# TrevorS/voxtral-mini-realtime-rs

Measured on AMD Instinct MI355X. Metric: decode_tok_per_s, higher is better.
Workload: dtype f32

## Files before the change

### include/voxtral_hip.h

```cpp
#ifndef VOXTRAL_HIP_H
#define VOXTRAL_HIP_H

#include <stddef.h>
#include <stdint.h>

#ifdef __cplusplus
extern "C" {
#endif

#define VOX_OK 0
#define VOX_ERR_INVALID 1
#define VOX_ERR_IO 2
#define VOX_ERR_HIP 3
#define VOX_ERR_NOTFOUND 4
#define VOX_ERR_UNSUPPORTED 5

#define VOX_MEM_HOST 0
#define VOX_MEM_DEVICE 1

typedef struct vox_ctx vox_ctx;
typedef struct vox_gguf vox_gguf;
typedef struct vox_q4 vox_q4;
typedef struct vox_model vox_model;
typedef struct vox_cache vox_cache;
// ... 14 lines not shown
int32_t vox_dev_download(vox_ctx* ctx, void* dst_host, const void* src_dev, size_t nbytes);
int32_t vox_dev_copy(vox_ctx* ctx, void* dst_dev, const void* src_dev, size_t nbytes);

int32_t vox_resample_len(size_t n_in, uint32_t sr_in, uint32_t sr_out, size_t* n_out);
int32_t vox_resample(vox_ctx* ctx, const float* in, size_t n_in, uint32_t sr_in, uint32_t sr_out, float* out, size_t cap, size_t* n_out,
                     int32_t mem_kind);
int32_t vox_resample_plan(uint32_t sr_in, uint32_t sr_out, int32_t* fft_in, int32_t* fft_out, int32_t* delay, float* cutoff, float* taps_or_null, size_t cap);
int32_t vox_peak_normalize(float* samples, size_t n, float target_peak);

typedef struct {
    uint32_t sample_rate;
    uint32_t n_left_pad_tokens;
    float    frame_rate;
    uint32_t extra_right_pad_tokens;
} vox_pad_cfg;
int32_t vox_pad_cfg_voxtral(vox_pad_cfg* cfg);
int32_t vox_pad_len(size_t n, const vox_pad_cfg* cfg, size_t* out);
int32_t vox_pad_audio(const float* in, size_t n, const vox_pad_cfg* cfg, float* out);
int32_t vox_num_audio_tokens(size_t n, const vox_pad_cfg* cfg, size_t* out);

typedef struct {
    uint32_t max_mel_frames;
    uint32_t hop_length;
    uint32_t sample_rate;
    uint32_t overlap_frames;
} vox_chunk_cfg;
typedef struct { size_t start_sample, end_sample, index; int32_t is_last; } vox_chunk;
int32_t vox_needs_chunking(size_t n, const vox_chunk_cfg* cfg, int32_t* out);
int32_t vox_chunk_plan(size_t n, const vox_chunk_cfg* cfg, vox_chunk* out, size_t cap, size_t* n_chunks);

int32_t vox_mel_num_frames(size_t n_samples, size_t* out);
int32_t vox_mel_filterbank(float* out_128x201);
int32_t vox_hann_window(int32_t length, float* out);
int32_t vox_mel_compute_log(vox_ctx* ctx, const float* samples, size_t n, float* out_Tx128, int32_t mem_kind);

int32_t vox_time_embedding(float t, int32_t dim, float* out);

int32_t vox_gguf_open(const char* path, vox_gguf** out);
int32_t vox_gguf_open_memory(const void* data, size_t size, vox_gguf** out);
int32_t vox_gguf_open_shards(const void* const* shards, const size_t* sizes, int32_t n, vox_gguf** out);
int32_t vox_gguf_close(vox_gguf* g);
int32_t vox_gguf_version(const vox_gguf* g, uint32_t* out);
int32_t vox_gguf_tensor_count(const vox_gguf* g, uint64_t* out);
int32_t vox_gguf_tensor_name(const vox_gguf* g, uint64_t index, const char** out);
int32_t vox_gguf_tensor_info(const vox_gguf* g, const char* name, uint64_t dims[4], uint32_t* ndims,
                             uint32_t* dtype, uint64_t* nbytes);
int32_t vox_gguf_tensor_data(const vox_gguf* g, const char* name, void* dst, size_t cap);

int32_t vox_q4_tensor_from_bytes(vox_ctx* ctx, const uint8_t* raw, size_t nbytes, int64_t N, int64_t K, vox_q4** out);
int32_t vox_q4_tensor_shape(const vox_q4* q, int64_t* N, int64_t* K);
int32_t vox_q4_tensor_num_blocks(const vox_q4* q, int64_t* out);
int32_t vox_q4_tensor_dequantize(vox_ctx* ctx, const vox_q4* q, float* out_NxK);
int32_t vox_q4_tensor_free(vox_q4* q);
int32_t vox_q4_matmul(vox_ctx* ctx, const vox_q4* w, const float* x, int32_t B, int32_t M, float* out, int32_t mem_kind);
int32_t vox_q4_linear_forward(vox_ctx* ctx, const vox_q4* w, const float* bias_or_null, const float* x,
                              int32_t B, int32_t M, float* out, int32_t mem_kind);

int32_t vox_dense_tensor_from_f32(vox_ctx* ctx, const float* w_NxK, const float* w_other_or_null, int64_t N, int64_t K, vox_q4** out);
int32_t vox_linear_forward_ex(vox_ctx* ctx, const vox_q4* w, const float* bias_or_null, const float* x, int32_t B, int32_t M, float* out, int32_t epilogue, int32_t mem_kind);
int32_t vox_conv_downsample(vox_ctx* ctx, const float* x_CxL, int32_t C, int32_t L, const float* w1, const float* b1, const float* w2, const float* b2, int32_t O, float* out_OxL2);

typedef struct {
    int32_t enc_layers, enc_dim, enc_heads, enc_head_dim, enc_ffn, enc_window;
    int32_t dec_layers, dec_dim, dec_heads, dec_kv_heads, dec_head_dim, dec_ffn, dec_window, vocab;
    int32_t n_mels, reshape_factor, t_cond_dim;
    float rope_theta, norm_eps;
} vox_model_cfg;

int32_t vox_attention(vox_ctx* ctx, const float* q, const float* k, const float* v, int32_t M, int32_t kv_len, int32_t n_heads,
                      int32_t n_kv_heads, int32_t head_dim, int32_t offset, int32_t window, float* out, int32_t mem_kind);

int32_t vox_q4_model_load(vox_ctx* ctx, const char* gguf_path, vox_model** out);
#define VOX_LOAD_LAYOUT_ONLY 1u
int32_t vox_q4_model_load_ex(vox_ctx* ctx, const char* gguf_path, uint32_t flags, vox_model** out);
int32_t vox_q4_model_load_gguf(vox_ctx* ctx, vox_gguf* g, uint32_t flags, vox_model** out);
int32_t vox_f32_model_load(vox_ctx* ctx, const char* safetensors_path, vox_model** out);
int32_t vox_model_free(vox_model* m);
int32_t vox_model_config(const vox_model* m, vox_model_cfg* out);
int32_t vox_model_weight_bytes(const vox_model* m, uint64_t* out);
int32_t vox_model_arena(const vox_model* m, void** dev_ptr, uint64_t* nbytes);
int32_t vox_model_arena_finalize(vox_model* m);
int32_t vox_model_replicate(const vox_model* src, vox_ctx* dst_ctx, vox_model** out);
int32_t vox_model_memory(const vox_model* m, uint64_t out[4]);

int32_t vox_model_set_t_embed(vox_model* m, const float* t_embed_host);
int32_t vox_model_set_decode_engine(vox_model* m, int32_t on, int32_t* active_or_null);
int32_t vox_model_set_prefix_cache(vox_model* m, int32_t on, int32_t* active_or_null);
int32_t vox_model_prefix_info(const vox_model* m, int32_t out[4]);
int32_t vox_model_set_batch_engine(vox_model* m, int32_t on, int32_t* active_or_null, uint64_t* launches_or_null);

int32_t vox_encode_audio(vox_model* m, const float* mel_128xT, int32_t T, float* out, int32_t cap_rows,
                         int32_t* S, int32_t mem_kind);
int32_t vox_transcribe_streaming(vox_model* m, const float* mel_128xT, int32_t T, const float* t_embed,
                                 int32_t* out_ids, int32_t cap, int32_t* n_ids, float* logits_or_null,
                                 int32_t mem_kind);
int32_t vox_transcribe_audio(vox_model* m, const float* samples, size_t n, const float* t_embed,
                             int32_t* out_ids, int32_t cap, int32_t* n_ids, int32_t mem_kind);

int32_t vox_transcribe_batch(vox_model* m, int32_t n, const float* const* samples, const size_t* n_samples, const float* t_embed,
                             int32_t* const* out_ids, const int32_t* caps, int32_t* n_ids, int32_t mem_kind);
int32_t vox_transcribe_batch_ex(vox_model* m, int32_t n, const float* const* samples, const size_t* n_samples, const int32_t* norm_group_or_null, const float* t_embed,
                                int32_t* const* out_ids, const int32_t* caps, int32_t* n_ids, int32_t mem_kind);
int32_t vox_model_set_sessions(vox_model* m, int32_t sessions);

int32_t vox_decoder_cache_create(vox_model* m, int32_t max_seq, vox_cache** out);
int32_t vox_cache_free(vox_cache* c);
int32_t vox_cache_seq_len(const vox_cache* c, int32_t* out);
int32_t vox_cache_reset(vox_cache* c);
int32_t vox_cache_update(vox_cache* c, int32_t layer, int32_t pos, const float* k_HxNxhd, const float* v_HxNxhd, int32_t n_rows, int32_t mem_kind);
int32_t vox_cache_truncate(vox_cache* c, int32_t len);
int32_t vox_encoder_cache_create(vox_model* m, int32_t capacity_rows, vox_cache** out);
int32_t vox_encoder_cache_apply_sliding_window(vox_cache* enc_cache, int32_t window);
int32_t vox_cache_abs_pos(const vox_cache* c, int32_t* out);
int32_t vox_encode_audio_with_cache(vox_model* m, const float* mel_128xT, int32_t T, vox_cache* enc_cache, float* out, int32_t cap_rows,
                                    int32_t* S, int32_t mem_kind);
int32_t vox_embed_tokens_from_ids(vox_model* m, const int32_t* ids, int32_t n, float* out_nxD);
int32_t vox_forward_hidden_with_cache(vox_model* m, const float* x_MxD, int32_t M, const float* t_embed,
                                      vox_cache* cache, float* out_MxD);
int32_t vox_lm_head(vox_model* m, const float* hidden_MxD, int32_t M, float* logits_MxV);
int32_t vox_embed_tokens_from_ids_ex(vox_model* m, const int32_t* ids_host, int32_t n, float* out_nxD, int32_t mem_kind);
int32_t vox_tensor_add(vox_ctx* ctx, const float* a, const float* b, size_t n, float* out, int32_t mem_kind);
int32_t vox_forward_hidden_with_cache_ex(vox_model* m, const float* x_MxD, int32_t M, const float* t_embed, vox_cache* cache, float* out_MxD_or_null,
                                         const float** hidden_ws_or_null, int32_t mem_kind);
int32_t vox_lm_head_ex(vox_model* m, const float* hidden_MxD, int32_t M, float* logits_MxV, int32_t mem_kind);
int32_t vox_argmax_rows(vox_ctx* ctx, const float* logits_MxV, int32_t M, int32_t V, int32_t* ids_host, int32_t mem_kind);
int32_t vox_lm_head_argmax(vox_model* m, const float* hidden_MxD, int32_t M, int32_t* ids_host, int32_t mem_kind);
int32_t vox_generate_step_with_cache(vox_model* m, const int32_t* token_ids, int32_t n, const float* t_embed, vox_cache* cache, float* logits_nxV);

int32_t vox_forward(vox_model* m, const float* mel_128xT, int32_t T, const float* t_embed, float* logits_SxV, int32_t cap_rows, int32_t* S, int32_t mem_kind);
int32_t vox_forward_streaming(vox_model* m, const float* mel_128xT, int32_t T, const int32_t* token_ids, int32_t n_ids, const float* t_embed, float* logits_SxV,
                              int32_t cap_rows, int32_t* S, int32_t mem_kind);
int32_t vox_forward_with_cache(vox_model* m, const float* mel_128xT, int32_t T, const float* t_embed, vox_cache* enc_cache, vox_cache* dec_cache, float* logits_SxV,
                               int32_t cap_rows, int32_t* S, int32_t mem_kind);

typedef struct { double preprocess_ms, encode_ms, decode_ms, total_ms; int32_t decode_tokens; int32_t graph_replays; } vox_timings;
int32_t vox_get_stage_timings(const vox_model* m, vox_timings* out);

int32_t vox_debug_reload_knobs(void);
int32_t vox_debug_attn_launches(uint64_t* out, int32_t cap);
int32_t vox_debug_gemm_launches(uint64_t* out, int32_t cap);
int32_t vox_debug_occupy(vox_ctx* ctx, int32_t workgroups, int32_t micros);

int32_t vox_bench_decode_gemv(vox_model* m, int32_t which, int32_t iters, double* avg_us, double* bytes_per_launch,
                              const char** kernel_name);

int32_t vox_bench_wide(vox_model* m, int32_t which, int32_t mt, int32_t iters, double out_us[4]);

int32_t vox_debug_timeline_start(vox_ctx* ctx, int32_t n_slots, int32_t n_waves);
int32_t vox_debug_timeline_fetch(vox_ctx* ctx, uint64_t* out, size_t cap_words, int32_t* slots_used, int32_t* meta );
int32_t vox_debug_batch_tap_arm(vox_model* m, const int32_t* units, int32_t n_units, int32_t max_rows);
int32_t vox_debug_batch_tap_fetch(vox_model* m, float* out, int32_t* rows_per_unit);
int32_t vox_debug_encode_batch(vox_model* m, int32_t n, const float* const* mels, const int32_t* T, int32_t layout, float* out, int64_t cap_rows,
                               int32_t* rows_per_clip, int64_t* report);
int32_t vox_debug_step_costs(const double base[9], const double meas[9], int32_t calib, int32_t shared, double out[9]);
int32_t vox_debug_plan_slots(const int32_t* steps, int32_t n, int32_t force_G, int32_t max_groups, const double step_ms[9], int32_t* G, int32_t* job_slot,
                             int32_t* job_qpos, int32_t steps_g[8], int32_t run_g[8], double* cost_ms);

typedef struct vox_stream vox_stream;
int32_t vox_stream_create(vox_model* m, const float* t_embed, float gain, int32_t enc_capacity_rows, int32_t max_positions, vox_stream** out);
int32_t vox_stream_push(vox_stream* s, const float* samples, size_t n, int32_t mem_kind, int32_t* out_ids, int32_t cap, int32_t* n_ids);
int32_t vox_stream_finish(vox_stream* s, int32_t* out_ids, int32_t cap, int32_t* n_ids);
int32_t vox_stream_reset(vox_stream* s);
int32_t vox_stream_free(vox_stream* s);
int32_t vox_stream_info(const vox_stream* s, int64_t out[8]);
int32_t vox_stream_schedule(size_t n_samples, int32_t finished, int32_t* positions, int32_t* ids);
int32_t vox_debug_stream_tap_arm(vox_stream* s, int32_t max_rows);
int32_t vox_debug_stream_tap_fetch(vox_stream* s, float* out_rows_x_vocab, int32_t* rows);

#ifdef __cplusplus
}
#endif
#endif
```

### voxtral-mini-realtime-rs_amd/_lib.py

```python
from __future__ import annotations

import ctypes as C
import os

from .build import LIB_PATH


class VoxError(RuntimeError):
    def __init__(self, code, msg):
        super().__init__(f"[vox error {code}] {msg}")
        self.code = code


class PadCfg(C.Structure):
    _fields_ = [("sample_rate", C.c_uint32), ("n_left_pad_tokens", C.c_uint32), ("frame_rate", C.c_float),
                ("extra_right_pad_tokens", C.c_uint32)]


class ChunkCfg(C.Structure):
    _fields_ = [("max_mel_frames", C.c_uint32), ("hop_length", C.c_uint32), ("sample_rate", C.c_uint32),
                ("overlap_frames", C.c_uint32)]


class Chunk(C.Structure):
    _fields_ = [("start_sample", C.c_size_t), ("end_sample", C.c_size_t), ("index", C.c_size_t), ("is_last", C.c_int32)]


class ModelCfg(C.Structure):
    _fields_ = [(n, C.c_int32) for n in ("enc_layers", "enc_dim", "enc_heads", "enc_head_dim", "enc_ffn", "enc_window",
                                         "dec_layers", "dec_dim", "dec_heads", "dec_kv_heads", "dec_head_dim", "dec_ffn",
                                         "dec_window", "vocab", "n_mels", "reshape_factor", "t_cond_dim")] + \
               [("rope_theta", C.c_float), ("norm_eps", C.c_float)]


class Timings(C.Structure):
    _fields_ = [("preprocess_ms", C.c_double), ("encode_ms", C.c_double), ("decode_ms", C.c_double), ("total_ms", C.c_double),
                ("decode_tokens", C.c_int32), ("graph_replays", C.c_int32)]


vp, i32, i64, u32, u64, sz, f32 = C.c_void_p, C.c_int32, C.c_int64, C.c_uint32, C.c_uint64, C.c_size_t, C.c_float
P = C.POINTER

SIGNATURES = {
    "vox_last_error": (C.c_char_p, []),
    "vox_abi_version": (i32, []),
    "vox_device_count": (i32, [P(i32)]),
    "vox_ctx_create": (i32, [i32, P(vp)]),
    "vox_ctx_destroy": (i32, [vp]),
    "vox_debug_reload_knobs": (i32, []),
    "vox_ctx_synchronize": (i32, [vp]),
    "vox_ctx_set_shared": (i32, [vp, i32]),
    "vox_ctx_stream": (i32, [vp, P(vp)]),
    "vox_dev_alloc": (i32, [vp, sz, P(vp)]),
    "vox_dev_free": (i32, [vp, vp]),
    "vox_dev_upload": (i32, [vp, vp, vp, sz]),
    "vox_dev_download": (i32, [vp, vp, vp, sz]),
    "vox_dev_copy": (i32, [vp, vp, vp, sz]),
    "vox_peak_normalize": (i32, [vp, sz, f32]),
    "vox_pad_cfg_voxtral": (i32, [P(PadCfg)]),
    "vox_pad_len": (i32, [sz, P(PadCfg), P(sz)]),
    "vox_pad_audio": (i32, [vp, sz, P(PadCfg), vp]),
    "vox_num_audio_tokens": (i32, [sz, P(PadCfg), P(sz)]),
    "vox_needs_chunking": (i32, [sz, P(ChunkCfg), P(i32)]),
    "vox_chunk_plan": (i32, [sz, P(ChunkCfg), P(Chunk), sz, P(sz)]),
    "vox_mel_num_frames": (i32, [sz, P(sz)]),
    "vox_mel_filterbank": (i32, [vp]),
    "vox_hann_window": (i32, [i32, vp]),
    "vox_mel_compute_log": (i32, [vp, vp, sz, vp, i32]),
    "vox_time_embedding": (i32, [f32, i32, vp]),
    "vox_gguf_open": (i32, [C.c_char_p, P(vp)]),
    "vox_gguf_open_memory": (i32, [vp, C.c_size_t, P(vp)]),
    "vox_gguf_open_shards": (i32, [vp, vp, i32, P(vp)]),
    "vox_q4_model_load_gguf": (i32, [vp, vp, C.c_uint32, P(vp)]),
    "vox_gguf_close": (i32, [vp]),
    "vox_gguf_version": (i32, [vp, P(u32)]),
    "vox_gguf_tensor_count": (i32, [vp, P(u64)]),
    "vox_gguf_tensor_name": (i32, [vp, u64, P(C.c_char_p)]),
    "vox_gguf_tensor_info": (i32, [vp, C.c_char_p, P(u64 * 4), P(u32), P(u32), P(u64)]),
    "vox_gguf_tensor_data": (i32, [vp, C.c_char_p, vp, sz]),
    "vox_q4_tensor_from_bytes": (i32, [vp, vp, sz, i64, i64, P(vp)]),
    "vox_q4_tensor_shape": (i32, [vp, P(i64), P(i64)]),
    "vox_q4_tensor_num_blocks": (i32, [vp, P(i64)]),
    "vox_q4_tensor_dequantize": (i32, [vp, vp, vp]),
    "vox_q4_tensor_free": (i32, [vp]),
    "vox_q4_matmul": (i32, [vp, vp, vp, i32, i32, vp, i32]),
    "vox_q4_linear_forward": (i32, [vp, vp, vp, vp, i32, i32, vp, i32]),
    "vox_dense_tensor_from_f32": (i32, [vp, vp, vp, i64, i64, P(vp)]),
    "vox_linear_forward_ex": (i32, [vp, vp, vp, vp, i32, i32, vp, i32, i32]),
    "vox_conv_downsample": (i32, [vp, vp, i32, i32, vp, vp, vp, vp, i32, vp]),
    "vox_attention": (i32, [vp, vp, vp, vp, i32, i32, i32, i32, i32, i32, i32, vp, i32]),
    "vox_q4_model_load": (i32, [vp, C.c_char_p, P(vp)]),
    "vox_q4_model_load_ex": (i32, [vp, C.c_char_p, u32, P(vp)]),
    "vox_f32_model_load": (i32, [vp, C.c_char_p, P(vp)]),
    "vox_model_free": (i32, [vp]),
    "vox_model_config": (i32, [vp, P(ModelCfg)]),
    "vox_model_weight_bytes": (i32, [vp, P(u64)]),
    "vox_model_arena": (i32, [vp, P(vp), P(u64)]),
    "vox_model_set_t_embed": (i32, [vp, vp]),
    "vox_model_set_decode_engine": (i32, [vp, i32, P(i32)]),
    "vox_model_set_prefix_cache": (i32, [vp, i32, P(i32)]),
    "vox_model_prefix_info": (i32, [vp, P(i32 * 4)]),
    "vox_debug_occupy": (i32, [vp, i32, i32]),
    "vox_model_memory": (i32, [vp, P(C.c_uint64)]),
    "vox_model_set_batch_engine": (i32, [vp, i32, P(i32), P(C.c_uint64)]),
    "vox_model_arena_finalize": (i32, [vp]),
    "vox_model_replicate": (i32, [vp, vp, P(vp)]),
    "vox_model_set_sessions": (i32, [vp, i32]),
    "vox_generate_step_with_cache": (i32, [vp, vp, i32, vp, vp, vp]),
    "vox_encode_audio": (i32, [vp, vp, i32, vp, i32, P(i32), i32]),
    "vox_transcribe_streaming": (i32, [vp, vp, i32, vp, vp, i32, P(i32), vp, i32]),
    "vox_transcribe_audio": (i32, [vp, vp, sz, vp, vp, i32, P(i32), i32]),
    "vox_transcribe_batch": (i32, [vp, i32, P(vp), P(sz), vp, P(vp), P(i32), P(i32), i32]),
    "vox_transcribe_batch_ex": (i32, [vp, i32, P(vp), P(sz), vp, vp, P(vp), P(i32), P(i32), i32]),
    "vox_decoder_cache_create": (i32, [vp, i32, P(vp)]),
    "vox_cache_free": (i32, [vp]),
    "vox_cache_seq_len": (i32, [vp, P(i32)]),
    "vox_cache_reset": (i32, [vp]),
    "vox_cache_update": (i32, [vp, i32, i32, vp, vp, i32, i32]),
    "vox_cache_truncate": (i32, [vp, i32]),
    "vox_resample_len": (i32, [sz, C.c_uint32, C.c_uint32, P(sz)]),
    "vox_resample": (i32, [vp, vp, sz, C.c_uint32, C.c_uint32, vp, sz, P(sz), i32]),
    "vox_resample_plan": (i32, [C.c_uint32, C.c_uint32, P(i32), P(i32), P(i32), P(C.c_float), vp, sz]),
    "vox_encoder_cache_create": (i32, [vp, i32, P(vp)]),
    "vox_encoder_cache_apply_sliding_window": (i32, [vp, i32]),
    "vox_cache_abs_pos": (i32, [vp, P(i32)]),
    "vox_encode_audio_with_cache": (i32, [vp, vp, i32, vp, vp, i32, P(i32), i32]),
    "vox_embed_tokens_from_ids": (i32, [vp, vp, i32, vp]),
    "vox_forward_hidden_with_cache": (i32, [vp, vp, i32, vp, vp, vp]),
    "vox_lm_head": (i32, [vp, vp, i32, vp]),
    "vox_embed_tokens_from_ids_ex": (i32, [vp, vp, i32, vp, i32]),
    "vox_tensor_add": (i32, [vp, vp, vp, sz, vp, i32]),
    "vox_forward_hidden_with_cache_ex": (i32, [vp, vp, i32, vp, vp, vp, P(vp), i32]),
    "vox_lm_head_ex": (i32, [vp, vp, i32, vp, i32]),
    "vox_argmax_rows": (i32, [vp, vp, i32, i32, vp, i32]),
    "vox_lm_head_argmax": (i32, [vp, vp, i32, vp, i32]),
    "vox_forward": (i32, [vp, vp, i32, vp, vp, i32, P(i32), i32]),
    "vox_forward_streaming": (i32, [vp, vp, i32, vp, i32, vp, vp, i32, P(i32), i32]),
    "vox_forward_with_cache": (i32, [vp, vp, i32, vp, vp, vp, vp, i32, P(i32), i32]),
    "vox_get_stage_timings": (i32, [vp, P(Timings)]),
    "vox_bench_decode_gemv": (i32, [vp, i32, i32, P(C.c_double), P(C.c_double), P(C.c_char_p)]),
    "vox_bench_wide": (i32, [vp, i32, i32, i32, P(C.c_double)]),
    "vox_debug_attn_launches": (i32, [P(C.c_uint64), i32]),
    "vox_debug_gemm_launches": (i32, [P(C.c_uint64), i32]),
    "vox_debug_timeline_start": (i32, [vp, i32, i32]),
    "vox_debug_timeline_fetch": (i32, [vp, vp, sz, P(i32), vp]),
    "vox_debug_batch_tap_arm": (i32, [vp, P(i32), i32, i32]),
    "vox_debug_batch_tap_fetch": (i32, [vp, vp, P(i32)]),
    "vox_debug_encode_batch": (i32, [vp, i32, P(vp), P(i32), i32, vp, C.c_int64, P(i32), P(C.c_int64)]),
    "vox_stream_create": (i32, [vp, vp, f32, i32, i32, P(vp)]),
    "vox_stream_push": (i32, [vp, vp, sz, i32, vp, i32, P(i32)]),
    "vox_stream_finish": (i32, [vp, vp, i32, P(i32)]),
    "vox_stream_reset": (i32, [vp]),
    "vox_stream_free": (i32, [vp]),
    "vox_stream_info": (i32, [vp, P(i64 * 8)]),
    "vox_debug_step_costs": (i32, [P(C.c_double), P(C.c_double), i32, i32, P(C.c_double)]),
    "vox_debug_plan_slots": (i32, [P(i32), i32, i32, i32, P(C.c_double), P(i32), P(i32), P(i32), P(i32), P(i32), P(C.c_double)]),
    "vox_stream_schedule": (i32, [sz, i32, P(i32), P(i32)]),
    "vox_debug_stream_tap_arm": (i32, [vp, i32]),
    "vox_debug_stream_tap_fetch": (i32, [vp, vp, P(i32)]),
}

_LIB = None
_KNOBS = None


def _knob_env():
    return tuple(sorted((k, v) for k, v in os.environ.items() if k.startswith("VOX_")))


def lib():
    global _LIB, _KNOBS
    if _LIB is not None:
        k = _knob_env()
        if k != _KNOBS:
            _KNOBS = k; _LIB.vox_debug_reload_knobs()
        return _LIB
    if not os.path.exists(LIB_PATH):
        raise VoxError(-1, f"{LIB_PATH} not built: run `python __graft_entry__.py build` (hipcc, gfx950). "
                           "There is no CPU fallback for the HIP path.")
    L = C.CDLL(LIB_PATH)
    for name, (res, args) in SIGNATURES.items():
        fn = getattr(L, name)
        fn.restype = res
        fn.argtypes = args
    _LIB = L; _KNOBS = _knob_env()
    return L
# ... 6 lines not shown
```

### voxtral-mini-realtime-rs_amd/csrc/vox_api.cpp

```cpp
#include "../../include/voxtral_hip.h"
#include "vox_kernels.h"

#include <dlfcn.h>
#include <fcntl.h>
#include <sys/mman.h>
#include <sys/stat.h>
#include <unistd.h>

#include <algorithm>
#include <cassert>
#include <chrono>
#include <cmath>
#include <cstdarg>
#include <cstdio>
#include <cstdlib>
#include <cstring>
#include <map>
#include <mutex>
#include <string>
#include <unordered_map>
#include <thread>
#include <vector>

using namespace vox;
// ... 413 lines not shown
    if (g) { if (g->map && g->own == 1) munmap(g->map, g->size); else if (g->map && g->own == 2) std::free(g->map); delete g; }
    return VOX_OK;
}
static int32_t gguf_parse(vox_gguf* g, vox_gguf** out) {
    Cur c{g->map, 0, g->size};
    const uint32_t magic = c.rd<uint32_t>();
    if (c.bad || magic != 0x46554747u) { vox_gguf_close(g); return fail(VOX_ERR_IO, "Invalid GGUF magic: 0x%08X (expected 0x46554747)", magic); }
    g->version = c.rd<uint32_t>();
    if (g->version != 2 && g->version != 3) { uint32_t v = g->version; vox_gguf_close(g); return fail(VOX_ERR_IO, "Unsupported GGUF version: %u (expected 2 or 3)", v); }
    const uint64_t nt = c.rd<uint64_t>(), nkv = c.rd<uint64_t>();
    for (uint64_t i = 0; i < nkv && !c.bad; i++) {
        (void)c.str(); const uint32_t ty = c.rd<uint32_t>();
        if (c.skip_value(ty)) { vox_gguf_close(g); return fail(VOX_ERR_IO, "Unknown GGUF metadata value type"); }
    }
    if (c.bad || nt > (1u << 24)) { vox_gguf_close(g); return fail(VOX_ERR_IO, "Failed to parse GGUF metadata"); }
    g->tensors.resize(nt);
    for (uint64_t i = 0; i < nt; i++) {
        GTensor& t = g->tensors[i];
        t.name = c.str(); t.ndims = c.rd<uint32_t>();
        if (c.bad || t.ndims > 4) { vox_gguf_close(g); return fail(VOX_ERR_IO, "Failed to read tensor %llu", (unsigned long long)i); }
        uint64_t ne = 1; bool ovf = false;
        for (uint32_t d = 0; d < t.ndims; d++) { t.dims[d] = c.rd<uint64_t>(); if (__builtin_mul_overflow(ne, t.dims[d], &ne)) ovf = true; }
        t.dtype = c.rd<uint32_t>(); t.offset = c.rd<uint64_t>();
        if (c.bad) { vox_gguf_close(g); return fail(VOX_ERR_IO, "Failed to read tensor %llu", (unsigned long long)i); }
        if (ovf || ne > (1ull << 60)) { std::string n = t.name; vox_gguf_close(g); return fail(VOX_ERR_IO, "tensor '%s' has an element count that overflows", n.c_str()); }
        if (t.dtype > 2) { uint32_t d = t.dtype; vox_gguf_close(g); return fail(VOX_ERR_IO, "Unsupported GGML dtype code: %u", d); }
        t.nbytes = t.dtype == 0 ? ne * 4 : t.dtype == 1 ? ne * 2 : (ne / 32) * 18;
        g->index[t.name] = i;
    }
    g->data_off = (c.pos + 31) / 32 * 32;
    for (auto& t : g->tensors) {
        uint64_t end = 0;
        if (g->data_off > g->size || __builtin_add_overflow(g->data_off, t.offset, &end) || __builtin_add_overflow(end, t.nbytes, &end) || end > g->size) {
            std::string n = t.name; vox_gguf_close(g); return fail(VOX_ERR_IO, "tensor '%s' exceeds file size", n.c_str());
        }
    }
    *out = g; return VOX_OK;
}
extern "C" int32_t vox_gguf_open(const char* path, vox_gguf** out) {
    ARGCHK(path && out, "null argument");
    int fd = open(path, O_RDONLY);
    if (fd < 0) return fail(VOX_ERR_IO, "cannot open %s: %s", path, strerror(errno));
    struct stat st;
    if (fstat(fd, &st) != 0 || st.st_size < 24) { close(fd); return fail(VOX_ERR_IO, "%s is not a GGUF file (stat failed or shorter than a header)", path); }
    void* mp = mmap(nullptr, st.st_size, PROT_READ, MAP_PRIVATE, fd, 0); close(fd);
    if (mp == MAP_FAILED) return fail(VOX_ERR_IO, "mmap of %s failed", path);
    vox_gguf* g = new vox_gguf(); g->map = (uint8_t*)mp; g->size = st.st_size; g->own = 1;
    return gguf_parse(g, out);
}
extern "C" int32_t vox_gguf_open_memory(const void* data, size_t size, vox_gguf** out) {
    ARGCHK(data && out, "null argument"); ARGCHK(size >= 24, "GGUF image too small (%zu bytes)", size);
    vox_gguf* g = new vox_gguf(); g->map = (uint8_t*)const_cast<void*>(data); g->size = size; g->own = 0;
    return gguf_parse(g, out);
}
extern "C" int32_t vox_gguf_open_shards(const void* const* shards, const size_t* sizes, int32_t n, vox_gguf** out) {
    ARGCHK(shards && sizes && out && n > 0, "bad shard list");
    size_t total = 0; for (int i = 0; i < n; i++) { ARGCHK(shards[i] || sizes[i] == 0, "null shard %d", i); total += sizes[i]; }
    ARGCHK(total >= 24, "GGUF image too small (%zu bytes)", total);
    uint8_t* buf = (uint8_t*)std::malloc(total); if (!buf) return fail(VOX_ERR_IO, "out of host memory for %zu bytes of shards", total);
    size_t o = 0; for (int i = 0; i < n; i++) { std::memcpy(buf + o, shards[i], sizes[i]); o += sizes[i]; }
    vox_gguf* g = new vox_gguf(); g->map = buf; g->size = total; g->own = 2;
    return gguf_parse(g, out);
}
extern "C" int32_t vox_gguf_version(const vox_gguf* g, uint32_t* out) { ARGCHK(g && out, "null argument"); *out = g->version; return VOX_OK; }
extern "C" int32_t vox_gguf_tensor_count(const vox_gguf* g, uint64_t* out) { ARGCHK(g && out, "null argument"); *out = g->tensors.size(); return VOX_OK; }
extern "C" int32_t vox_gguf_tensor_name(const vox_gguf* g, uint64_t i, const char** out) {
    ARGCHK(g && out, "null argument"); ARGCHK(i < g->tensors.size(), "tensor index out of range"); *out = g->tensors[i].name.c_str(); return VOX_OK;
}
extern "C" int32_t vox_gguf_tensor_info(const vox_gguf* g, const char* name, uint64_t dims[4], uint32_t* ndims, uint32_t* dtype, uint64_t* nbytes) {
    ARGCHK(g && name && dims && ndims && dtype && nbytes, "null argument");
    const GTensor* t = g->find(name);
    if (!t) return fail(VOX_ERR_NOTFOUND, "Tensor '%s' not found in GGUF", name);
    for (uint32_t d = 0; d < 4; d++) dims[d] = d < t->ndims ? t->dims[d] : 0;
    *ndims = t->ndims; *dtype = t->dtype; *nbytes = t->nbytes; return VOX_OK;
}
extern "C" int32_t vox_gguf_tensor_data(const vox_gguf* g, const char* name, void* dst, size_t cap) {
    ARGCHK(g && name && dst, "null argument");
    const GTensor* t = g->find(name);
    if (!t) return fail(VOX_ERR_NOTFOUND, "Tensor '%s' not found in GGUF", name);
    ARGCHK(cap >= t->nbytes, "destination too small for '%s' (%zu < %llu)", name, cap, (unsigned long long)t->nbytes);
    std::memcpy(dst, g->data(t), t->nbytes); return VOX_OK;
}

struct vox_q4 { vox_ctx* ctx; Q4W w; void* qs_mem; void* sc_mem; void* qt_mem = nullptr; void* st_mem = nullptr; };

static int32_t upload_repack(vox_ctx* c, const uint8_t* raw, int64_t n_blocks, int nb, uint4* qs, uint16_t* sc, int row_mul, int row_add,
                             void* staging, size_t staging_cap) {
    const size_t bytes = (size_t)n_blocks * 18;
    DevBuf tmp; uint8_t* d_raw = (uint8_t*)staging;
    if (!staging || staging_cap < bytes) { HIPCHK(tmp.alloc(bytes)); d_raw = tmp.as<uint8_t>(); }
    HIPCHK(hipMemcpyAsync(d_raw, raw, bytes, hipMemcpyHostToDevice, c->stream));
    HIPCHK(launch_q4_repack(d_raw, qs, sc, n_blocks, nb, row_mul, row_add, c->stream));
    HIPCHK(hipStreamSynchronize(c->stream));
    return VOX_OK;
}

extern "C" int32_t vox_q4_tensor_from_bytes(vox_ctx* c, const uint8_t* raw, size_t nbytes, int64_t N, int64_t K, vox_q4** out) {
    ARGCHK(c && raw && out, "null argument"); ARGCHK(N > 0 && K > 0, "bad shape"); VOXCHK(ctx_bind(c));
    const int64_t ne = N * K;
    ARGCHK(ne % 32 == 0, "Q4_0 requires element count divisible by 32, got %lld", (long long)ne);
    const int64_t nblk = ne / 32;
    ARGCHK((int64_t)nbytes == nblk * 18, "Q4_0 byte count mismatch: expected %lld for %lld blocks, got %zu", (long long)(nblk * 18), (long long)nblk, nbytes);
    ARGCHK(K % 32 == 0, "Q4_0 rows must be a whole number of 32-element blocks (K=%lld)", (long long)K);
    vox_q4* q = new vox_q4(); q->ctx = c; q->qs_mem = q->sc_mem = nullptr;
    if (hipMalloc(&q->qs_mem, (size_t)nblk * 16) != hipSuccess || hipMalloc(&q->sc_mem, (size_t)nblk * 2) != hipSuccess) {
        if (q->qs_mem) (void)hipFree(q->qs_mem); delete q; return fail(VOX_ERR_HIP, "hipMalloc failed for Q4 tensor");
    }
    q->w = Q4W{(const uint4*)q->qs_mem, (const uint16_t*)q->sc_mem, (int)N, (int)K, (int)(K / 32)};
    int32_t r = upload_repack(c, raw, nblk, (int)(K / 32), (uint4*)q->qs_mem, (uint16_t*)q->sc_mem, 1, 0, nullptr, 0);
    if (r != VOX_OK) { (void)hipFree(q->qs_mem); (void)hipFree(q->sc_mem); delete q; return r; }
    if ((K / 32) % 4 == 0) {
        const size_t n_tiles = (size_t)(N + 15) / 16, nq = (size_t)(K / 128);
        if (hipMalloc(&q->qt_mem, n_tiles * nq * 64 * 16) == hipSuccess && hipMalloc(&q->st_mem, n_tiles * nq * 64 * 2) == hipSuccess &&
            launch_q4_tile_build(q->w, (uint4*)q->qt_mem, (uint16_t*)q->st_mem, c->stream) == hipSuccess && hipStreamSynchronize(c->stream) == hipSuccess) {
            q->w.qt = (const uint4*)q->qt_mem; q->w.st = (const uint16_t*)q->st_mem;
        } else { (void)hipFree(q->qt_mem); (void)hipFree(q->st_mem); (void)hipFree(q->qs_mem); (void)hipFree(q->sc_mem); delete q; return fail(VOX_ERR_HIP, "tile copy of Q4 tensor failed"); }
    }
    *out = q; return VOX_OK;
}
extern "C" int32_t vox_q4_tensor_shape(const vox_q4* q, int64_t* N, int64_t* K) { ARGCHK(q && N && K, "null argument"); *N = q->w.N; *K = q->w.K; return VOX_OK; }
extern "C" int32_t vox_q4_tensor_num_blocks(const vox_q4* q, int64_t* out) { ARGCHK(q && out, "null argument"); *out = (int64_t)q->w.N * q->w.nb; return VOX_OK; }
extern "C" int32_t vox_q4_tensor_free(vox_q4* q) {
    if (!q) return VOX_OK;
    (void)hipSetDevice(q->ctx->device); (void)hipStreamSynchronize(q->ctx->stream);
    (void)hipFree(q->qs_mem); (void)hipFree(q->sc_mem); (void)hipFree(q->qt_mem); (void)hipFree(q->st_mem); delete q; return VOX_OK;
}
extern "C" int32_t vox_q4_tensor_dequantize(vox_ctx* c, const vox_q4* q, float* out) {
    ARGCHK(c && q && out, "null argument"); VOXCHK(ctx_bind(c));
    const size_t ne = (size_t)q->w.N * q->w.K;
    DevBuf d; HIPCHK(d.alloc(ne * 4));
    HIPCHK(launch_q4_dequant(q->w, d.as<float>(), c->stream));
    HIPCHK(hipMemcpyAsync(out, d.p, ne * 4, hipMemcpyDeviceToHost, c->stream)); HIPCHK(hipStreamSynchronize(c->stream));
    return VOX_OK;
}

static int32_t q4_linear_dev(vox_ctx* c, const Q4W& w, const float* bias, const float* x, int x_stride, int rows, float* out, int out_stride,
                             int epi = EPI_STORE, const float* resid = nullptr, int resid_stride = 0, int ksplit = 0) {
    if (rows <= 4) {
        GemvParams p{}; p.w = w; p.x = x; p.x_stride = x_stride; p.out = out; p.out_stride = out_stride; p.bias = bias;
        p.resid = resid; p.resid_stride = resid_stride;
        HIPCHK(launch_q4_gemv(p, rows, PRO_NONE, epi, q4_gemv_default_R(w.N, w.K, epi), c->stream));
    } else {
        GemmParams p{}; p.w = w; p.x = x; p.x_stride = x_stride; p.M = rows; p.out = out; p.out_stride = out_stride; p.bias = bias;
        p.resid = resid; p.resid_stride = resid_stride; p.ksplit = ksplit;
        if (rows > 16 && rows <= 48 && w.fmt == WFMT_Q4_0 && w.K <= 16384) {
            c->want_scratch(true, true);
            p.xf_scratch = c->xf_scratch; p.xf_scratch_bytes = c->xf_scratch_bytes;
            p.kz_scratch = c->kz_scratch; p.kz_scratch_bytes = c->kz_scratch_bytes;
        }
        HIPCHK(launch_q4_gemm(p, epi, c->stream));
    }
    return VOX_OK;
}

extern "C" int32_t vox_q4_linear_forward(vox_ctx* c, const vox_q4* w, const float* bias, const float* x, int32_t B, int32_t M, float* out, int32_t mem_kind) {
    ARGCHK(c && w && x && out, "null argument"); ARGCHK(B > 0 && M > 0, "bad batch/rows"); VOXCHK(ctx_bind(c));
    const int rows = B * M, K = w->w.K, N = w->w.N;
    if (mem_kind == VOX_MEM_DEVICE) return q4_linear_dev(c, w->w, bias, x, K, rows, out, N);
    DevBuf dx, dy, db; HIPCHK(dx.alloc((size_t)rows * K * 4)); HIPCHK(dy.alloc((size_t)rows * N * 4));
    HIPCHK(hipMemcpyAsync(dx.p, x, (size_t)rows * K * 4, hipMemcpyHostToDevice, c->stream));
    if (bias) { HIPCHK(db.alloc((size_t)N * 4)); HIPCHK(hipMemcpyAsync(db.p, bias, (size_t)N * 4, hipMemcpyHostToDevice, c->stream)); }
    VOXCHK(q4_linear_dev(c, w->w, bias ? db.as<float>() : nullptr, dx.as<float>(), K, rows, dy.as<float>(), N));
    HIPCHK(hipMemcpyAsync(out, dy.p, (size_t)rows * N * 4, hipMemcpyDeviceToHost, c->stream)); HIPCHK(hipStreamSynchronize(c->stream));
    return VOX_OK;
}
extern "C" int32_t vox_q4_matmul(vox_ctx* c, const vox_q4* w, const float* x, int32_t B, int32_t M, float* out, int32_t mem_kind) {
    return vox_q4_linear_forward(c, w, nullptr, x, B, M, out, mem_kind);
}

static uint16_t bf16_rne(float f) { uint32_t u; std::memcpy(&u, &f, 4); return (uint16_t)((u + 0x7FFFu + ((u >> 16) & 1u)) >> 16); }
static void bf16_split(const float* w, size_t n, uint16_t* hi, uint16_t* lo) {
    for (size_t e = 0; e < n; e++) { const uint16_t hb = bf16_rne(w[e]); const uint32_t hu = (uint32_t)hb << 16; float hf; std::memcpy(&hf, &hu, 4); hi[e] = hb; lo[e] = bf16_rne(w[e] - hf); }
}
extern "C" int32_t vox_dense_tensor_from_f32(vox_ctx* c, const float* w, const float* w_other, int64_t N, int64_t K, vox_q4** out) {
    ARGCHK(c && w && out, "null argument"); ARGCHK(N > 0 && K > 0 && K % 32 == 0, "dense tensor [%lld][%lld]: K must be a positive multiple of 32", (long long)N, (long long)K);
    VOXCHK(ctx_bind(c));
    const int64_t Ntot = w_other ? 2 * N : N; const size_t ne = (size_t)Ntot * K;
    std::vector<float> host(ne);
    for (int64_t r = 0; r < N; r++) {
        std::memcpy(host.data() + (size_t)(w_other ? 2 * r : r) * K, w + (size_t)r * K, (size_t)K * 4);
        if (w_other) std::memcpy(host.data() + (size_t)(2 * r + 1) * K, w_other + (size_t)r * K, (size_t)K * 4);
    }
    std::vector<uint16_t> h2(ne), l2(ne); bf16_split(host.data(), ne, h2.data(), l2.data());
    vox_q4* q = new vox_q4{c, Q4W{}, nullptr, nullptr};
    auto bail = [&](hipError_t e) { (void)hipGetLastError(); (void)hipFree(q->qs_mem); (void)hipFree(q->sc_mem); (void)hipFree(q->qt_mem); delete q; return fail(VOX_ERR_HIP, "dense tensor upload: %s", hipGetErrorString(e)); };
    hipError_t e = hipMalloc(&q->qs_mem, ne * 2); if (e == hipSuccess) e = hipMalloc(&q->sc_mem, ne * 2); if (e == hipSuccess) e = hipMalloc(&q->qt_mem, ne * 4);
    if (e == hipSuccess) e = hipMemcpy(q->qs_mem, h2.data(), ne * 2, hipMemcpyHostToDevice);
    if (e == hipSuccess) e = hipMemcpy(q->sc_mem, l2.data(), ne * 2, hipMemcpyHostToDevice);
    if (e == hipSuccess) e = hipMemcpy(q->qt_mem, host.data(), ne * 4, hipMemcpyHostToDevice);
    if (e != hipSuccess) return bail(e);
    q->w = Q4W{(const uint4*)q->qs_mem, (const uint16_t*)q->sc_mem, (int)Ntot, (int)K, (int)(K / 32), WFMT_F32}; q->w.qt = (const uint4*)q->qt_mem;
    *out = q; return VOX_OK;
}
extern "C" int32_t vox_linear_forward_ex(vox_ctx* c, const vox_q4* w, const float* bias, const float* x, int32_t B, int32_t M, float* out, int32_t epilogue, int32_t mem_kind) {
    ARGCHK(c && w && x && out, "null argument"); ARGCHK(B > 0 && M > 0, "bad batch/rows"); VOXCHK(ctx_bind(c));
    ARGCHK(epilogue == 0 || epilogue == 1 || epilogue == 2, "epilogue %d: 0 none, 1 GELU, 2 SwiGLU over interleaved gate / up rows", epilogue);
    const int epi = epilogue == 1 ? EPI_GELU : epilogue == 2 ? EPI_SWIGLU : EPI_STORE;
    const int rows = B * M, K = w->w.K, N = w->w.N, No = epilogue == 2 ? N / 2 : N;
    ARGCHK(epilogue != 2 || (N % 2 == 0 && !bias), "SwiGLU epilogue needs an even number of interleaved rows and no bias");
    if (mem_kind == VOX_MEM_DEVICE) return q4_linear_dev(c, w->w, bias, x, K, rows, out, No, epi);
    DevBuf dx, dy, db; HIPCHK(dx.alloc((size_t)rows * K * 4)); HIPCHK(dy.alloc((size_t)rows * No * 4));
    HIPCHK(hipMemcpyAsync(dx.p, x, (size_t)rows * K * 4, hipMemcpyHostToDevice, c->stream));
    if (bias) { HIPCHK(db.alloc((size_t)N * 4)); HIPCHK(hipMemcpyAsync(db.p, bias, (size_t)N * 4, hipMemcpyHostToDevice, c->stream)); }
    VOXCHK(q4_linear_dev(c, w->w, bias ? db.as<float>() : nullptr, dx.as<float>(), K, rows, dy.as<float>(), No, epi));
    HIPCHK(hipMemcpyAsync(out, dy.p, (size_t)rows * No * 4, hipMemcpyDeviceToHost, c->stream)); HIPCHK(hipStreamSynchronize(c->stream));
    return VOX_OK;
}
extern "C" int32_t vox_conv_downsample(vox_ctx* c, const float* x, int32_t C, int32_t L, const float* w1, const float* b1, const float* w2, const float* b2, int32_t O, float* out) {
// ... 17 lines not shown
    HIPCHK(launch_transpose(dx.as<float>(), C, L, dm.as<float>() + C, s));
    { GemmParams g{}; g.w = g1; g.x = dm.as<float>(); g.x_stride = 2 * C; g.M = T1; g.out = d1.as<float>() + O; g.out_stride = O; g.bias = db1.as<float>(); HIPCHK(launch_dense2_gemm(g, EPI_GELU, s)); }
    { GemmParams g{}; g.w = g2; g.x = d1.as<float>(); g.x_stride = 2 * O; g.M = S; g.out = dy.as<float>(); g.out_stride = O; g.bias = db2.as<float>(); HIPCHK(launch_dense2_gemm(g, EPI_GELU, s)); }
    HIPCHK(launch_transpose(dy.as<float>(), S, O, dyt.as<float>(), s));
    HIPCHK(hipMemcpyAsync(out, dyt.p, (size_t)S * O * 4, hipMemcpyDeviceToHost, s)); HIPCHK(hipStreamSynchronize(s));
    return VOX_OK;
}

extern "C" int32_t vox_attention(vox_ctx* c, const float* q, const float* k, const float* v, int32_t M, int32_t kv_len, int32_t n_heads,
                                 int32_t n_kv_heads, int32_t head_dim, int32_t offset, int32_t window, float* out, int32_t mem_kind) {
    ARGCHK(c && q && k && v && out, "null argument");
    ARGCHK(M > 0 && kv_len > 0 && n_heads > 0 && n_kv_heads > 0 && n_heads % n_kv_heads == 0, "bad attention shape");
    ARGCHK(head_dim == 64 || head_dim == 128, "head_dim must be 64 (encoder) or 128 (decoder)");
    ARGCHK(offset >= 0 && offset + M <= kv_len, "queries must lie inside the key range (offset + M <= kv_len)");
    VOXCHK(ctx_bind(c));
    const size_t qn = (size_t)M * n_heads * head_dim, kn = (size_t)kv_len * n_kv_heads * head_dim;
    DevBuf dq, dk, dv, dout;
    const float *pq = q, *pk = k, *pv = v; float* po = out;
    if (mem_kind != VOX_MEM_DEVICE) {
        HIPCHK(dq.alloc(qn * 4)); HIPCHK(dk.alloc(kn * 4)); HIPCHK(dv.alloc(kn * 4)); HIPCHK(dout.alloc(qn * 4));
        HIPCHK(hipMemcpyAsync(dq.p, q, qn * 4, hipMemcpyHostToDevice, c->stream));
        HIPCHK(hipMemcpyAsync(dk.p, k, kn * 4, hipMemcpyHostToDevice, c->stream));
        HIPCHK(hipMemcpyAsync(dv.p, v, kn * 4, hipMemcpyHostToDevice, c->stream));
        pq = dq.as<float>(); pk = dk.as<float>(); pv = dv.as<float>(); po = dout.as<float>();
    }
    AttnParams ap{}; ap.q = pq; ap.q_stride = n_heads * head_dim; ap.k = pk; ap.v = pv; ap.kv_row_stride = n_kv_heads * head_dim; ap.kv_head_stride = head_dim;
    ap.out = po; ap.out_stride = n_heads * head_dim; ap.M = M; ap.kv_len = kv_len; ap.n_heads = n_heads; ap.n_kv_heads = n_kv_heads; ap.offset = offset; ap.window = window;
    HIPCHK(launch_attn_prefill(ap, head_dim, c->stream));
    if (mem_kind != VOX_MEM_DEVICE) { HIPCHK(hipMemcpyAsync(out, po, qn * 4, hipMemcpyDeviceToHost, c->stream)); HIPCHK(hipStreamSynchronize(c->stream)); }
    return VOX_OK;
}

struct Lin { Q4W w{}; const float* bias = nullptr; };
struct EncLayer { const float *attn_norm = nullptr, *ffn_norm = nullptr; Lin wqkv, wo, w13, w2; };
struct DecLayer { const float *attn_norm = nullptr, *ffn_norm = nullptr; Lin wqkv, wo, w13, w2, ada0, ada2; float* ada_mul = nullptr; };

struct vox_cache { vox_model* m; vox_ctx* ctx = nullptr; float *k = nullptr, *v = nullptr; int max_seq = 0, len = 0; size_t layer_stride = 0;
                   int kind = 0, abs_pos = 0; uint64_t gen = 0; };

static std::mutex g_cache_mu; static std::unordered_map<const vox_cache*, uint64_t> g_cache_live; static uint64_t g_cache_gen = 0;
static void cache_register(vox_cache* k) { std::lock_guard<std::mutex> l(g_cache_mu); k->gen = ++g_cache_gen; g_cache_live[k] = k->gen; }
static void cache_unregister(const vox_cache* k) { std::lock_guard<std::mutex> l(g_cache_mu); g_cache_live.erase(k); }
static bool cache_alive(const vox_cache* k, uint64_t gen) { std::lock_guard<std::mutex> l(g_cache_mu); auto it = g_cache_live.find(k); return it != g_cache_live.end() && it->second == gen; }
static void cache_release(vox_cache*& k) { if (!k) return; cache_unregister(k); (void)hipFree(k->k); (void)hipFree(k->v); delete k; k = nullptr; }

struct EngBinding {
    EngLayerTab* tab = nullptr; float* part_val = nullptr; int* part_idx = nullptr; unsigned* err_word = nullptr; const vox_cache* cache = nullptr; uint64_t gen = 0; std::vector<EngLayerTab> host;
};
static void binding_release(EngBinding& b) {
    for (void* p : {(void*)b.tab, (void*)b.part_val, (void*)b.part_idx}) if (p) (void)hipFree(p);
    if (b.err_word) (void)hipHostFree(b.err_word);
    b = EngBinding{};
}

struct TensorMeta { std::vector<uint64_t> shape; int dtype = 0; uint64_t nbytes = 0; };
struct PrefixState {
    bool on = true;
    int RC = 0, PC = 0;
    float* enc_kv = nullptr;
    float* audio = nullptr;
    float *dec_k = nullptr, *dec_v = nullptr;
    bool enc_built = false, dec_built = false;
    std::vector<float> t_embed;
    float* capture = nullptr; int capture_rows = 0;
    uint64_t enc_bytes = 0, dec_bytes = 0;
};
static const int VOX_PREFIX_TOKENS = 38, VOX_TOK_BOS = 1, VOX_TOK_STREAMING_PAD = 32;
static const struct PrefixTokens {
    int32_t t[VOX_PREFIX_TOKENS];
    PrefixTokens() { std::fill(t, t + VOX_PREFIX_TOKENS, VOX_TOK_STREAMING_PAD); t[0] = VOX_TOK_BOS; }
} PREFIX_TOKENS;
enum class StepLaunch { StepAndArgmax, EngineAlone, EngineArgmaxFirst };
struct DecodeGraphs {
    struct Key { const vox_cache* cache; const float* audio; int unroll; StepLaunch launch; } key{nullptr, nullptr, 0, StepLaunch::StepAndArgmax};
    hipGraph_t graph[2] = {nullptr, nullptr}; hipGraphExec_t exec[2] = {nullptr, nullptr};
};
struct vox_model {
    PrefixState pfx;
    vox_ctx* ctx = nullptr; vox_model_cfg cfg{};
    std::vector<vox_model*> twins;
    std::map<std::string, TensorMeta> manifest; bool is_q4 = false;
    uint8_t* arena = nullptr; uint64_t arena_bytes = 0, arena_primary_bytes = 0;
    std::vector<Q4W*> tiled;
    const float *conv1_w = nullptr, *conv1_b = nullptr, *conv2_w = nullptr, *conv2_b = nullptr, *enc_norm = nullptr, *dec_norm = nullptr;
    Q4W conv1_g{}, conv2_g{};
    const float *enc_cos = nullptr, *enc_sin = nullptr, *dec_cos = nullptr, *dec_sin = nullptr;
    int enc_rope_len = 4096, dec_rope_len = 16384;
    std::vector<EncLayer> enc; std::vector<DecLayer> dec; Lin ad0, ad2, tok;
    float* ada_mul = nullptr; bool t_embed_set = false; std::vector<float> t_embed_host;
    float* ws = nullptr; size_t ws_floats = 0;
    float *d_audio = nullptr; int audio_cap = 0;
    float *d_mel = nullptr; size_t mel_cap = 0;
    float *d_samples = nullptr; size_t samples_cap = 0;
    vox_cache* cache = nullptr;
    int *d_tokens = nullptr, *d_pos = nullptr; int tokens_cap = 0;
    float* d_prefix = nullptr;
    float *enc_cos_s = nullptr, *enc_sin_s = nullptr; int enc_rope_s_len = 0;
    int* d_seq_len = nullptr; std::vector<int> h_seq_len;
    int *d_seq_off = nullptr, *d_row_pos = nullptr; size_t row_pos_cap = 0; std::vector<int> h_seq_off, h_row_pos;
    float *d_h = nullptr, *d_q = nullptr, *d_att = nullptr, *d_act = nullptr, *d_logits = nullptr, *d_part_val = nullptr; int* d_part_idx = nullptr;
    float* d_h2 = nullptr; long long* d_wo_acc = nullptr;
    int n_parts = 0, argmax_R = 8;
    bool eng_ok = false, eng_on = true, eng_ready = false; unsigned char* eng_stream = nullptr; unsigned char* eng_state = nullptr; unsigned long long eng_launches = 0;
    EngBinding eng_offline, eng_pw;
    int eng_flags = 128 | 512 | 1, eng_pace = 50;
    int eng_strikes = 0; bool eng_suspended = false;
    unsigned char* eng_wob = nullptr;
    bool engb_ok = false; unsigned char* engb_state[4] = {nullptr, nullptr, nullptr, nullptr}; EngLayerTab* engb_tab[4] = {nullptr, nullptr, nullptr, nullptr};
    bool engb_on = true; unsigned long long engb_launches = 0; int engb_strikes = 0;
    int batch_sessions = 0;
    int engb_flags = 128 | 1 | 64 | 2048;
    int engb_flags2 = 128 | 1024;
    unsigned engb_err_host[4][2] = {{0, 0}, {0, 0}, {0, 0}, {0, 0}};
    DecodeGraphs graphs;
    float *pw_x = nullptr, *pw_hidden = nullptr, *pw_logits = nullptr; size_t pw_x_cap = 0, pw_hidden_cap = 0, pw_logits_cap = 0;
    int* pw_ids = nullptr; int pw_ids_cap = 0; int* pw_zero = nullptr;
    bool pw_memo = false, pw_eng_used = false;
    vox_cache* pw_pend_cache = nullptr; uint64_t pw_pend_gen = 0; int pw_pend_rows = 0; bool pw_verdict_failed = false;
    vox_timings timings{};
    struct { std::vector<int> units; int max_rows = 0; bool armed = false, on = false, ready = false; float* out = nullptr; int* rows = nullptr; } tap;
};

struct Arena {
    uint8_t* base = nullptr; uint64_t off = 0;
    template <class T> T* take(size_t count) {
        off = (off + 255) / 256 * 256;
        T* p = base ? reinterpret_cast<T*>(base + off) : nullptr;
        off += count * sizeof(T);
        return p;
    }
};

#define ENC_PFX "mm_streams_embeddings.embedding_module.whisper_encoder"
#define EMB_PFX "mm_streams_embeddings.embedding_module"
#define TOK_NAME EMB_PFX ".tok_embeddings.weight"
#define ADP_PFX EMB_PFX ".audio_language_projection"

enum { DT_F32 = 0, DT_F16 = 1, DT_Q4_0 = 2, DT_BF16 = 3 };
struct TensorView { std::vector<uint64_t> shape; int dtype = 0; const uint8_t* data = nullptr; uint64_t nbytes = 0; };
struct TensorSource {
    virtual ~TensorSource() {}
    virtual bool find(const std::string& name, TensorView* out) const = 0;
    virtual uint64_t max_q4_bytes() const { return 0; }
};
struct GgufSource : TensorSource {
    vox_gguf* g = nullptr;
    ~GgufSource() override { if (g) vox_gguf_close(g); }
    bool find(const std::string& name, TensorView* out) const override {
        const GTensor* t = g->find(name); if (!t) return false;
        out->shape.assign(t->dims, t->dims + t->ndims); std::reverse(out->shape.begin(), out->shape.end());
        out->dtype = (int)t->dtype; out->data = g->data(t); out->nbytes = t->nbytes; return true;
    }
    uint64_t max_q4_bytes() const override { uint64_t m = 0; for (auto& t : g->tensors) if (t.dtype == 2) m = std::max<uint64_t>(m, t.nbytes); return m; }
};
struct RecordingSource : TensorSource {
    const TensorSource* in; mutable std::map<std::string, TensorMeta> seen;
    explicit RecordingSource(const TensorSource* s) : in(s) {}
    bool find(const std::string& name, TensorView* out) const override { if (!in->find(name, out)) return false; TensorMeta& t = seen[name]; t.shape = out->shape; t.dtype = out->dtype; t.nbytes = out->nbytes; return true; }
    uint64_t max_q4_bytes() const override { return in->max_q4_bytes(); }
};
struct ManifestSource : TensorSource {
    const std::map<std::string, TensorMeta>* m;
    bool find(const std::string& name, TensorView* out) const override { auto it = m->find(name); if (it == m->end()) return false; out->shape = it->second.shape; out->dtype = it->second.dtype; out->data = nullptr; out->nbytes = it->second.nbytes; return true; }
};
struct SafeTensorsSource : TensorSource {
    uint8_t* map = nullptr; size_t size = 0; std::map<std::string, TensorView> tensors;
// ... 47 lines not shown
                    skip_ws(p, e); if (p >= e || *p != ':') return fail(VOX_ERR_IO, "bad SafeTensors entry"); p++;
                    if (key == "dtype") { if (!parse_string(p, e, &dt)) return fail(VOX_ERR_IO, "bad dtype"); have_dt = true; }
                    else if (key == "shape" || key == "data_offsets") {
                        skip_ws(p, e); if (p >= e || *p != '[') return fail(VOX_ERR_IO, "bad array"); p++;
                        std::vector<uint64_t> v;
                        for (;;) { skip_ws(p, e); if (p < e && *p == ']') { p++; break; } char* q; v.push_back(strtoull(p, &q, 10)); if (q == p) return fail(VOX_ERR_IO, "bad number"); p = q; skip_ws(p, e); if (p < e && *p == ',') p++; }
                        if (key == "shape") { tv.shape = v; have_shape = true; } else { if (v.size() != 2) return fail(VOX_ERR_IO, "bad data_offsets"); off[0] = v[0]; off[1] = v[1]; have_off = true; }
                    } else if (!skip_value(p, e)) return fail(VOX_ERR_IO, "bad SafeTensors value");
                    skip_ws(p, e); if (p < e && *p == ',') p++;
                }
                if (!have_dt || !have_off || !have_shape) return fail(VOX_ERR_IO, "incomplete SafeTensors entry '%s'", name.c_str());
                if (dt == "F32") tv.dtype = DT_F32; else if (dt == "F16") tv.dtype = DT_F16; else if (dt == "BF16") tv.dtype = DT_BF16;
                else return fail(VOX_ERR_UNSUPPORTED, "Unsupported dtype %s for tensor '%s'", dt.c_str(), name.c_str());
                if (off[1] < off[0] || off[1] > dsize) return fail(VOX_ERR_IO, "tensor '%s' exceeds file size", name.c_str());
                uint64_t ne = 1; for (auto d : tv.shape) ne *= d;
                if (off[1] - off[0] != ne * (tv.dtype == DT_F32 ? 4 : 2)) return fail(VOX_ERR_IO, "tensor '%s' byte size does not match its shape", name.c_str());
                tv.data = data0 + off[0]; tv.nbytes = off[1] - off[0]; tensors[name] = tv;
            }
            skip_ws(p, e); if (p < e && *p == ',') p++;
        }
        return VOX_OK;
    }
};

static float half_bits_to_f32(uint16_t x) {
    const uint32_t sign = (uint32_t)(x & 0x8000u) << 16; uint32_t e = (x >> 10) & 0x1f, man = x & 0x3ffu, bits;
    if (e == 0) { if (!man) bits = sign; else { int k = -1; do { man <<= 1; k++; } while (!(man & 0x400u)); bits = sign | ((uint32_t)(112 - k) << 23) | ((man & 0x3ffu) << 13); } }
    else if (e == 31) bits = sign | 0x7f800000u | (man << 13); else bits = sign | ((e + 112) << 23) | (man << 13);
    float f; std::memcpy(&f, &bits, 4); return f;
}
static void to_f32(const TensorView& t, uint64_t ne, float* out) {
    if (t.dtype == DT_F32) std::memcpy(out, t.data, ne * 4);
    else if (t.dtype == DT_F16) { const uint16_t* h = (const uint16_t*)t.data; for (uint64_t i = 0; i < ne; i++) out[i] = half_bits_to_f32(h[i]); }
    else { const uint16_t* h = (const uint16_t*)t.data; for (uint64_t i = 0; i < ne; i++) { const uint32_t b = (uint32_t)h[i] << 16; std::memcpy(&out[i], &b, 4); } }
}

namespace {
struct Loader {
    vox_model* m; const TensorSource* src; Arena ar; bool fill; void* staging = nullptr; size_t staging_cap = 0;
    Arena ar2;
    std::map<std::string, bool>* fmt_cache = nullptr;
    std::string err;

    bool setfail(const std::string& e) { if (err.empty()) err = e; return false; }
    bool need(const std::string& name, TensorView* t) { if (!src->find(name, t)) return setfail("Tensor '" + name + "' not found"); return true; }
    static uint64_t numel(const TensorView& t) { uint64_t n = 1; for (auto d : t.shape) n *= d; return n; }

    const float* f32(const std::string& name, bool required = true) {
        TensorView t;
        if (!src->find(name, &t)) { if (required) setfail("Tensor '" + name + "' not found"); return nullptr; }
        if (t.dtype == DT_Q4_0) { setfail("Cannot load Q4_0 tensor '" + name + "' as f32"); return nullptr; }
        const uint64_t ne = numel(t);
        float* dst = ar.take<float>(ne);
        if (fill) {
            std::vector<float> tmp(ne); to_f32(t, ne, tmp.data());
            if (hipMemcpy(dst, tmp.data(), ne * 4, hipMemcpyHostToDevice) != hipSuccess) setfail("hipMemcpy failed for '" + name + "'");
        }
        return dst;
    }
    bool conv_planes(const std::string& name, Q4W* out) {
        TensorView t; if (!need(name, &t)) return false;
        if (t.dtype == DT_Q4_0 || t.shape.size() != 3 || t.shape[2] != 3) return setfail("conv weight '" + name + "' must be a dense [out][in][3] tensor");
        const int64_t Co = (int64_t)t.shape[0], Ci = (int64_t)t.shape[1], K = 3 * Ci;
        if (K % 128) return setfail("conv weight '" + name + "': 3*Cin must be a multiple of 128");
        uint16_t* hi = ar.take<uint16_t>((size_t)Co * K); uint16_t* lo = ar.take<uint16_t>((size_t)Co * K);
        *out = Q4W{(const uint4*)hi, lo, (int)Co, (int)K, (int)(K / 32), WFMT_BF16X2};
        if (fill) {
            const uint64_t ne = numel(t); std::vector<float> w(ne); to_f32(t, ne, w.data());
            std::vector<uint16_t> h((size_t)Co * K), l((size_t)Co * K);
            auto rne = [](float f) { uint32_t u; std::memcpy(&u, &f, 4); return (uint16_t)((u + 0x7FFFu + ((u >> 16) & 1u)) >> 16); };
            for (int64_t co = 0; co < Co; co++)
                for (int64_t ci = 0; ci < Ci; ci++)
                    for (int kk = 0; kk < 3; kk++) {
                        const float v = w[(size_t)(co * Ci + ci) * 3 + kk];
                        const uint16_t hb = rne(v); const uint32_t hu = (uint32_t)hb << 16; float hf; std::memcpy(&hf, &hu, 4);
                        const size_t d = (size_t)co * K + (size_t)kk * Ci + ci;
                        h[d] = hb; l[d] = rne(v - hf);
                    }
            if (hipMemcpy(hi, h.data(), h.size() * 2, hipMemcpyHostToDevice) != hipSuccess || hipMemcpy(lo, l.data(), l.size() * 2, hipMemcpyHostToDevice) != hipSuccess)
                return setfail("hipMemcpy failed for conv planes");
        }
        return true;
    }
    bool lin(const std::vector<std::string>& parts, bool interleave, Lin* L, bool require_q4, bool tile = true) {
        int64_t K = -1, Ntot = 0; std::vector<TensorView> ts; int kind = -1;
        for (auto& n : parts) {
            TensorView t; if (!need(n, &t)) return false;
            if (require_q4 && t.dtype != DT_Q4_0) return setfail("Expected Q4_0 for '" + n + "'");
            if (t.shape.size() != 2) return setfail("Tensor '" + n + "' is not 2-D");
            const int64_t nn = (int64_t)t.shape[0], k = (int64_t)t.shape[1];
            if (k % 32) return setfail("tensor '" + n + "' has an inner dimension not divisible by 32");
            if (K < 0) K = k; else if (K != k) return setfail("fused tensors disagree on K");
            if (interleave && !ts.empty() && nn != (int64_t)ts[0].shape[0]) return setfail("interleaved tensors disagree on N");
            const int kd = t.dtype == DT_Q4_0 ? 0 : 1;
            if (kind < 0) kind = kd; else if (kind != kd) return setfail("fused tensors mix Q4_0 and dense dtypes");
            Ntot += nn; ts.push_back(t);
        }
        const int nb = (int)(K / 32);
        if (kind == 0) {
            uint4* qs = ar.take<uint4>((size_t)Ntot * nb); uint16_t* sc = ar.take<uint16_t>((size_t)Ntot * nb);
            L->w = Q4W{qs, sc, (int)Ntot, (int)K, nb, WFMT_Q4_0};
            if (fill) {
                int64_t row0 = 0;
                for (size_t i = 0; i < ts.size(); i++) {
                    const int64_t nn = (int64_t)ts[i].shape[0];
                    const int mul = interleave ? (int)ts.size() : 1, add = interleave ? (int)i : (int)row0;
                    if (upload_repack(m->ctx, ts[i].data, nn * nb, nb, qs, sc, mul, add, staging, staging_cap) != VOX_OK) return setfail(g_err);
                    row0 += nn;
                }
            }
            if (tile && nb % 4 == 0) {
                const size_t n_tiles = (size_t)(Ntot + 15) / 16, nq = (size_t)nb / 4;
                uint4* qt = ar2.take<uint4>(n_tiles * nq * 64); uint16_t* st = ar2.take<uint16_t>(n_tiles * nq * 64);
                L->w.qt = qt; L->w.st = st;
                if (ar2.base) m->tiled.push_back(&L->w);
                if (fill) {
                    if (launch_q4_tile_build(L->w, qt, st, m->ctx->stream) != hipSuccess || hipStreamSynchronize(m->ctx->stream) != hipSuccess)
                        return setfail("q4_tile_build failed");
                }
            }
            return true;
        }
        bool exact_bf16 = true;
        {
            auto it = fmt_cache->find(parts[0]);
            if (it != fmt_cache->end()) exact_bf16 = it->second;
            else {
                for (size_t i = 0; i < ts.size() && exact_bf16; i++) {
                    if (ts[i].dtype == DT_BF16) continue;
                    const uint64_t ne = numel(ts[i]);
                    if (ts[i].dtype == DT_F32) { const uint32_t* b = (const uint32_t*)ts[i].data; for (uint64_t e = 0; e < ne; e++) if (b[e] & 0xFFFFu) { exact_bf16 = false; break; } }
                    else { const uint16_t* h = (const uint16_t*)ts[i].data; for (uint64_t e = 0; e < ne; e++) { const float f = half_bits_to_f32(h[e]); uint32_t b; std::memcpy(&b, &f, 4); if (b & 0xFFFFu) { exact_bf16 = false; break; } } }
                }
                (*fmt_cache)[parts[0]] = exact_bf16;
            }
        }
        if (!exact_bf16) {
            float* wf = ar.take<float>((size_t)Ntot * K); uint16_t* hi = ar.take<uint16_t>((size_t)Ntot * K); uint16_t* lo = ar.take<uint16_t>((size_t)Ntot * K);
            L->w = Q4W{(const uint4*)hi, lo, (int)Ntot, (int)K, nb, WFMT_F32}; L->w.qt = (const uint4*)wf;
            if (fill) {
                std::vector<float> host((size_t)Ntot * K); std::vector<uint16_t> h2((size_t)Ntot * K), l2((size_t)Ntot * K);
                auto rne = [](float f) { uint32_t u; std::memcpy(&u, &f, 4); return (uint16_t)((u + 0x7FFFu + ((u >> 16) & 1u)) >> 16); };
                int64_t row0 = 0;
                for (size_t i = 0; i < ts.size(); i++) {
                    const int64_t nn = (int64_t)ts[i].shape[0];
                    std::vector<float> src((size_t)nn * K); to_f32(ts[i], (uint64_t)nn * K, src.data());
                    for (int64_t r = 0; r < nn; r++)
                        std::memcpy(host.data() + (size_t)(interleave ? r * (int64_t)ts.size() + (int64_t)i : row0 + r) * K, src.data() + (size_t)r * K, (size_t)K * 4);
                    row0 += nn;
                }
                for (size_t e = 0; e < host.size(); e++) { const uint16_t hb = rne(host[e]); const uint32_t hu = (uint32_t)hb << 16; float hf; std::memcpy(&hf, &hu, 4); h2[e] = hb; l2[e] = rne(host[e] - hf); }
                if (hipMemcpy(wf, host.data(), host.size() * 4, hipMemcpyHostToDevice) != hipSuccess || hipMemcpy(hi, h2.data(), h2.size() * 2, hipMemcpyHostToDevice) != hipSuccess ||
                    hipMemcpy(lo, l2.data(), l2.size() * 2, hipMemcpyHostToDevice) != hipSuccess) return setfail("hipMemcpy failed for dense f32 weight");
            }
            return true;
        }
        uint16_t* w = ar.take<uint16_t>((size_t)Ntot * K);
        L->w = Q4W{(const uint4*)w, nullptr, (int)Ntot, (int)K, nb, WFMT_BF16};
        if (fill) {
            std::vector<uint16_t> host((size_t)Ntot * K);
            int64_t row0 = 0;
            for (size_t i = 0; i < ts.size(); i++) {
                const int64_t nn = (int64_t)ts[i].shape[0];
                for (int64_t r = 0; r < nn; r++) {
                    uint16_t* dst = host.data() + (size_t)(interleave ? r * (int64_t)ts.size() + (int64_t)i : row0 + r) * K;
                    if (ts[i].dtype == DT_BF16) std::memcpy(dst, (const uint16_t*)ts[i].data + (size_t)r * K, (size_t)K * 2);
                    else {
                        for (int64_t k = 0; k < K; k++) {
                            float f = ts[i].dtype == DT_F32 ? ((const float*)ts[i].data)[(size_t)r * K + k] : half_bits_to_f32(((const uint16_t*)ts[i].data)[(size_t)r * K + k]);
                            uint32_t b; std::memcpy(&b, &f, 4);
                            if (b & 0xFFFFu) return setfail("internal: dense weight '" + parts[i] + "' was classified bf16-exact but is not");
                            dst[k] = (uint16_t)(b >> 16);
                        }
                    }
                }
                row0 += nn;
            }
            if (hipMemcpy(w, host.data(), host.size() * 2, hipMemcpyHostToDevice) != hipSuccess) return setfail("hipMemcpy failed for dense weight");
        }
        return true;
    }
    const float* bias_cat(const std::vector<std::pair<std::string, int64_t>>& parts) {
        bool any = false; int64_t tot = 0; TensorView t;
        for (auto& p : parts) { if (!p.first.empty() && src->find(p.first, &t)) any = true; tot += p.second; }
        if (!any) return nullptr;
        float* dst = ar.take<float>(tot);
        if (fill) {
            std::vector<float> host(tot, 0.0f); int64_t o = 0;
            for (auto& p : parts) {
                if (!p.first.empty() && src->find(p.first, &t)) {
                    if (t.dtype == DT_Q4_0 || (int64_t)numel(t) != p.second) setfail("bias '" + p.first + "' has the wrong dtype or size");
                    else to_f32(t, (uint64_t)p.second, host.data() + o);
                }
                o += p.second;
            }
            if (hipMemcpy(dst, host.data(), (size_t)tot * 4, hipMemcpyHostToDevice) != hipSuccess) setfail("hipMemcpy failed for bias");
        }
        return dst;
    }
    const float* rope(int hd, int len, float theta, bool sine) {
        const int half = hd / 2; float* dst = ar.take<float>((size_t)len * half);
        if (fill) {
            std::vector<float> t((size_t)len * half);
            for (int i = 0; i < len; i++)
                for (int j = 0; j < half; j++) {
                    const float inv = 1.0f / std::pow(theta, (float)(2 * j) / (float)hd), fr = (float)i * inv;
                    t[(size_t)i * half + j] = sine ? std::sin(fr) : std::cos(fr);
                }
            if (hipMemcpy(dst, t.data(), t.size() * 4, hipMemcpyHostToDevice) != hipSuccess) setfail("hipMemcpy failed for rope table");
        }
        return dst;
    }

    bool run(bool q4) {
        vox_model_cfg& c = m->cfg; char a[320]; TensorView tv;
        c.enc_head_dim = 64; c.dec_head_dim = 128; c.enc_window = 750; c.dec_window = 8192; c.rope_theta = 1e6f; c.norm_eps = 1e-5f; c.reshape_factor = 4;
        int ne = 0, nd = 0;
        for (;; ne++) { snprintf(a, sizeof a, ENC_PFX ".transformer.layers.%d.attention.wq.weight", ne); if (!src->find(a, &tv)) break; }
        for (;; nd++) { snprintf(a, sizeof a, "layers.%d.attention.wq.weight", nd); if (!src->find(a, &tv)) break; }
        if (ne == 0 || nd == 0) return setfail("model file has no encoder/decoder layers");
        c.enc_layers = ne; c.dec_layers = nd; m->enc.resize(ne); m->dec.resize(nd);
        TensorView cw; if (!need(ENC_PFX ".conv_layers.0.conv.weight", &cw)) return false;
        if (cw.shape.size() != 3 || cw.shape[2] != 3) return setfail("conv weight must be [out][in][3]");
        c.n_mels = (int)cw.shape[1]; c.enc_dim = (int)cw.shape[0];
        m->conv1_w = f32(ENC_PFX ".conv_layers.0.conv.weight"); m->conv1_b = f32(ENC_PFX ".conv_layers.0.conv.bias");
        m->conv2_w = f32(ENC_PFX ".conv_layers.1.conv.weight"); m->conv2_b = f32(ENC_PFX ".conv_layers.1.conv.bias");
        if ((3 * c.n_mels) % 128 == 0 && (3 * c.enc_dim) % 128 == 0) {
            if (!conv_planes(ENC_PFX ".conv_layers.0.conv.weight", &m->conv1_g) || !conv_planes(ENC_PFX ".conv_layers.1.conv.weight", &m->conv2_g)) return false;
        }
        for (int i = 0; i < ne; i++) {
            EncLayer& L = m->enc[i]; std::string p = std::string(ENC_PFX ".transformer.layers.") + std::to_string(i);
            L.attn_norm = f32(p + ".attention_norm.weight"); L.ffn_norm = f32(p + ".ffn_norm.weight");
            if (!lin({p + ".attention.wq.weight", p + ".attention.wk.weight", p + ".attention.wv.weight"}, false, &L.wqkv, q4)) return false;
            const int64_t hq = L.wqkv.w.N / 3;
            L.wqkv.bias = bias_cat({{p + ".attention.wq.bias", hq}, {"", hq}, {p + ".attention.wv.bias", hq}});
            if (!lin({p + ".attention.wo.weight"}, false, &L.wo, q4)) return false;
            L.wo.bias = bias_cat({{p + ".attention.wo.bias", L.wo.w.N}});
            if (!lin({p + ".feed_forward.w1.weight", p + ".feed_forward.w3.weight"}, true, &L.w13, q4)) return false;
            if (!lin({p + ".feed_forward.w2.weight"}, false, &L.w2, q4)) return false;
            L.w2.bias = bias_cat({{p + ".feed_forward.w2.bias", L.w2.w.N}});
        }
        m->enc_norm = f32(ENC_PFX ".transformer.norm.weight");
        if (!lin({ADP_PFX ".0.weight"}, false, &m->ad0, q4) || !lin({ADP_PFX ".2.weight"}, false, &m->ad2, q4)) return false;
        if (!lin({TOK_NAME}, false, &m->tok, false, true)) return false;
        for (int i = 0; i < nd; i++) {
            DecLayer& L = m->dec[i]; std::string p = "layers." + std::to_string(i);
            if (!lin({p + ".ada_rms_norm_t_cond.0.weight"}, false, &L.ada0, q4) || !lin({p + ".ada_rms_norm_t_cond.2.weight"}, false, &L.ada2, q4)) return false;
            L.attn_norm = f32(p + ".attention_norm.weight"); L.ffn_norm = f32(p + ".ffn_norm.weight");
            if (!lin({p + ".attention.wq.weight", p + ".attention.wk.weight", p + ".attention.wv.weight"}, false, &L.wqkv, q4, true)) return false;
            if (!lin({p + ".attention.wo.weight"}, false, &L.wo, q4, true)) return false;
            if (!lin({p + ".feed_forward.w1.weight", p + ".feed_forward.w3.weight"}, true, &L.w13, q4, true)) return false;
            if (!lin({p + ".feed_forward.w2.weight"}, false, &L.w2, q4, true)) return false;
        }
        m->dec_norm = f32("norm.weight");
        if (!err.empty()) return false;
        TensorView ewq, dwq, dwk;
        need(std::string(ENC_PFX ".transformer.layers.0.attention.wq.weight"), &ewq); need("layers.0.attention.wq.weight", &dwq); need("layers.0.attention.wk.weight", &dwk);
        c.enc_heads = (int)(ewq.shape[0] / c.enc_head_dim); c.enc_ffn = m->enc[0].w13.w.N / 2;
        c.dec_dim = (int)dwq.shape[1]; c.dec_heads = (int)(dwq.shape[0] / c.dec_head_dim); c.dec_kv_heads = (int)(dwk.shape[0] / c.dec_head_dim);
        c.dec_ffn = m->dec[0].w13.w.N / 2; c.vocab = m->tok.w.N; c.t_cond_dim = m->dec[0].ada0.w.N;
        if (ewq.shape[0] % c.enc_head_dim || dwq.shape[0] % c.dec_head_dim || dwk.shape[0] % c.dec_head_dim || c.dec_kv_heads == 0 || c.dec_heads % c.dec_kv_heads)
            return setfail("attention projection shapes are not multiples of head_dim");
        if ((int)ewq.shape[1] != c.enc_dim || m->ad0.w.K != c.enc_dim * c.reshape_factor || m->ad2.w.N != c.dec_dim || m->ad0.w.N != m->ad2.w.K || m->tok.w.K != c.dec_dim)
            return setfail("inconsistent encoder / adapter / embedding shapes");
        if (c.enc_dim % 32 || c.dec_dim % 32) return setfail("model dims must be multiples of 32");
        m->enc_cos = rope(c.enc_head_dim, m->enc_rope_len, c.rope_theta, false); m->enc_sin = rope(c.enc_head_dim, m->enc_rope_len, c.rope_theta, true);
        m->dec_cos = rope(c.dec_head_dim, m->dec_rope_len, c.rope_theta, false); m->dec_sin = rope(c.dec_head_dim, m->dec_rope_len, c.rope_theta, true);
        return err.empty();
    }
};
}

static void graphs_destroy(vox_model* m) {
    DecodeGraphs& g = m->graphs;
    for (int i = 0; i < 2; i++) {
        if (g.exec[i]) { (void)hipGraphExecDestroy(g.exec[i]); g.exec[i] = nullptr; }
        if (g.graph[i]) { (void)hipGraphDestroy(g.graph[i]); g.graph[i] = nullptr; }
    }
}
static void prefix_release(vox_model* m) {
    PrefixState& p = m->pfx;
    for (float** q : {&p.enc_kv, &p.audio, &p.dec_k, &p.dec_v}) { if (*q) (void)hipFree(*q); *q = nullptr; }
    p.enc_built = p.dec_built = false; p.enc_bytes = p.dec_bytes = 0; p.t_embed.clear();
}
static void model_release(vox_model* m) {
    if (!m) return;
    for (vox_model* t : m->twins) { vox_ctx* tc = t->ctx; model_release(t); (void)vox_ctx_destroy(tc); }
    m->twins.clear();
    (void)hipSetDevice(m->ctx->device); (void)hipStreamSynchronize(m->ctx->stream);
    graphs_destroy(m);
    cache_release(m->cache);
    if (m->ctx->pw_model == m) m->ctx->pw_model = nullptr;
    for (void* p : std::initializer_list<void*>{m->arena, m->ada_mul, m->ws, m->d_audio, m->d_mel, m->d_samples, m->d_tokens, m->d_pos, m->d_h, m->d_h2, m->d_wo_acc, m->d_q, m->d_att, m->d_act,
                    m->d_logits, m->d_part_val, m->d_part_idx, m->d_seq_len, m->d_seq_off, m->d_row_pos, m->d_prefix, m->enc_cos_s, m->enc_sin_s, m->eng_stream, m->eng_wob, m->eng_state,
                    m->engb_state[0], m->engb_state[1], m->engb_state[2], m->engb_state[3], m->engb_tab[0], m->engb_tab[1], m->engb_tab[2], m->engb_tab[3], m->pw_x, m->pw_hidden, m->pw_logits,
                    m->pw_ids, m->pw_zero, m->tap.out, m->tap.rows}) if (p) (void)hipFree(p);
    prefix_release(m);
    m->eng_offline.part_val = nullptr; m->eng_offline.part_idx = nullptr;
    binding_release(m->eng_offline); binding_release(m->eng_pw);
    delete m;
}
extern "C" int32_t vox_model_free(vox_model* m) { model_release(m); return VOX_OK; }

static int32_t model_build(vox_ctx* ctx, const TensorSource* src_in, bool q4, bool layout_only, vox_model** out) {
    vox_model* m = new vox_model(); m->ctx = ctx;
    RecordingSource rec(src_in); const TensorSource* src = &rec;
    std::map<std::string, bool> fmt_cache;
    Loader plan{m, src, Arena{}, false}; plan.fmt_cache = &fmt_cache;
    if (!plan.run(q4)) { std::string e = plan.err; model_release(m); return fail(VOX_ERR_IO, "%s", e.c_str()); }
    m->arena_primary_bytes = (plan.ar.off + 255) / 256 * 256 + 256;
    m->arena_bytes = m->arena_primary_bytes + plan.ar2.off + 256;
    if (hipMalloc((void**)&m->arena, m->arena_bytes) != hipSuccess) { model_release(m); return fail(VOX_ERR_HIP, "hipMalloc of %.1f MB weight arena failed", m->arena_bytes / 1e6); }
    const size_t max_q4 = layout_only ? 16 : std::max<uint64_t>(src->max_q4_bytes(), 16);
    DevBuf staging; if (staging.alloc(max_q4) != hipSuccess) { model_release(m); return fail(VOX_ERR_HIP, "hipMalloc of staging buffer failed"); }
    Loader fillr{m, src, Arena{m->arena, 0}, !layout_only, staging.p, max_q4}; fillr.fmt_cache = &fmt_cache; fillr.ar2 = Arena{m->arena + m->arena_primary_bytes, 0};
    if (!fillr.run(q4)) { std::string e = fillr.err; model_release(m); return fail(VOX_ERR_IO, "%s", e.c_str()); }
    const vox_model_cfg& c = m->cfg;
    const int qdim = c.dec_heads * c.dec_head_dim;
    if (m->tok.w.fmt == WFMT_BF16 || m->tok.w.fmt == WFMT_F32) { m->argmax_R = 2; m->n_parts = dense_gemv_grid(c.vocab); }
    else { m->argmax_R = q4_gemv_default_R(c.vocab, c.dec_dim, EPI_ARGMAX); m->n_parts = m->argmax_R > 0 ? q4_gemv_grid(c.vocab, m->argmax_R) : 1; }
    hipError_t e = hipSuccess;
    auto A = [&](void** p, size_t n) { if (e == hipSuccess) e = hipMalloc(p, n); };
    A((void**)&m->ada_mul, (size_t)c.dec_layers * c.dec_dim * 4); A((void**)&m->d_pos, 64); A((void**)&m->d_h, (size_t)c.dec_dim * 4 * 4);
    A((void**)&m->d_q, (size_t)qdim * 4 * 4); A((void**)&m->d_att, (size_t)qdim * 4 * 4); A((void**)&m->d_act, (size_t)c.dec_ffn * 4 * 4);
    A((void**)&m->d_h2, (size_t)c.dec_dim * 4); A((void**)&m->d_wo_acc, (size_t)c.dec_layers * c.dec_dim * 8);
    A((void**)&m->d_logits, (size_t)c.vocab * 4); A((void**)&m->d_part_val, (size_t)m->n_parts * 4 * 4); A((void**)&m->d_part_idx, (size_t)m->n_parts * 4 * 4);
    if (e != hipSuccess) { model_release(m); return fail(VOX_ERR_HIP, "hipMalloc of decode buffers failed: %s", hipGetErrorString(e)); }
    m->eng_offline.part_val = m->d_part_val; m->eng_offline.part_idx = m->d_part_idx;
    if (hipMemset(m->d_wo_acc, 0, (size_t)c.dec_layers * c.dec_dim * 8) != hipSuccess) { model_release(m); return fail(VOX_ERR_HIP, "hipMemset failed"); }
    for (int i = 0; i < c.dec_layers; i++) m->dec[i].ada_mul = m->ada_mul + (size_t)i * c.dec_dim;
    {
        const char* ev = knob_str("VOX_ENGINE"); bool ok = !(ev && ev[0] == '0') && c.dec_layers <= 32 && eng_geometry_ok(c.dec_dim, c.dec_heads, c.dec_kv_heads, c.dec_head_dim, c.dec_ffn, c.vocab, 256);
        hipDeviceProp_t prop; if (ok && (hipGetDeviceProperties(&prop, ctx->device) != hipSuccess || prop.multiProcessorCount != 256)) ok = false;
        for (int i = 0; ok && i < c.dec_layers; i++) { const DecLayer& L = m->dec[i]; for (const Lin* w : {&L.wqkv, &L.wo, &L.w13, &L.w2}) if (w->w.fmt != WFMT_Q4_0 || !w->w.qs || !w->w.sc || w->bias) ok = false; }
        if (ok && (m->tok.w.fmt != WFMT_Q4_0 || !m->tok.w.qs)) ok = false;
        if (ok) { int occ = 0; if (eng_occupancy(&occ) != hipSuccess || occ < 1) { ok = false; (void)hipGetLastError(); } }
        m->eng_ok = ok; m->eng_on = ok;
        {
            const char* bv = knob_str("VOX_BATCH_ENGINE"); int occ = 0;
            m->engb_ok = ok && !(bv && bv[0] == '0') && engb_occupancy(&occ) == hipSuccess && occ >= 1;
            (void)hipGetLastError();
            if (const char* f = knob_str("VOX_BATCH_ENGINE_FLAGS")) m->engb_flags = atoi(f);
            if (const char* f = knob_str("VOX_BATCH_ENGINE_FLAGS2")) m->engb_flags2 = atoi(f);
        }
        if (const char* f = knob_str("VOX_ENGINE_FLAGS")) m->eng_flags = atoi(f);
        if (const char* f = knob_str("VOX_ENGINE_PACE")) m->eng_pace = atoi(f);
    }
    m->manifest = std::move(rec.seen); m->is_q4 = q4;
    *out = m; return VOX_OK;
}

extern "C" int32_t vox_q4_model_load(vox_ctx* ctx, const char* path, vox_model** out) { return vox_q4_model_load_ex(ctx, path, 0, out); }

extern "C" int32_t vox_q4_model_load_gguf(vox_ctx* ctx, vox_gguf* g, uint32_t flags, vox_model** out) {
    ARGCHK(ctx && g && out, "null argument"); VOXCHK(ctx_bind(ctx));
    GgufSource src; src.g = g;
    const int32_t r = model_build(ctx, &src, true, (flags & VOX_LOAD_LAYOUT_ONLY) != 0, out);
    src.g = nullptr;
    return r;
}
extern "C" int32_t vox_q4_model_load_ex(vox_ctx* ctx, const char* path, uint32_t flags, vox_model** out) {
    ARGCHK(ctx && path && out, "null argument"); VOXCHK(ctx_bind(ctx));
    GgufSource src; VOXCHK(vox_gguf_open(path, &src.g));
    return model_build(ctx, &src, true, (flags & VOX_LOAD_LAYOUT_ONLY) != 0, out);
}

extern "C" int32_t vox_f32_model_load(vox_ctx* ctx, const char* path, vox_model** out) {
    ARGCHK(ctx && path && out, "null argument"); VOXCHK(ctx_bind(ctx));
    SafeTensorsSource src; VOXCHK(src.open(path));
    return model_build(ctx, &src, false, false, out);
}

extern "C" int32_t vox_model_config(const vox_model* m, vox_model_cfg* out) { ARGCHK(m && out, "null argument"); *out = m->cfg; return VOX_OK; }
extern "C" int32_t vox_model_weight_bytes(const vox_model* m, uint64_t* out) { ARGCHK(m && out, "null argument"); *out = m->arena_bytes; return VOX_OK; }
extern "C" int32_t vox_model_memory(const vox_model* m, uint64_t out[4]) {
    ARGCHK(m && out, "null argument");
    out[0] = m->arena_bytes; out[1] = m->arena_primary_bytes;
    out[2] = (m->eng_stream ? eng_stream_bytes(m->cfg.dec_layers, m->cfg.vocab) : 0) + (m->eng_wob ? engb_wo_stream_bytes(m->cfg.dec_layers) : 0);
    out[3] = m->eng_state ? eng_state_bytes() : 0;
    for (int gi = 0; gi < 4; gi++) if (m->engb_state[gi]) out[3] += engb_state_bytes();
    return VOX_OK;
}
extern "C" int32_t vox_model_arena(const vox_model* m, void** p, uint64_t* n) { ARGCHK(m && p && n, "null argument"); *p = m->arena; *n = m->arena_primary_bytes; return VOX_OK; }
extern "C" int32_t vox_model_arena_finalize(vox_model* m) {
    ARGCHK(m, "null argument"); VOXCHK(ctx_bind(m->ctx));
    for (Q4W* w : m->tiled) HIPCHK(launch_q4_tile_build(*w, const_cast<uint4*>(w->qt), const_cast<uint16_t*>(w->st), m->ctx->stream));
    HIPCHK(hipStreamSynchronize(m->ctx->stream));
    m->eng_ready = false; m->eng_offline.cache = nullptr;
    prefix_release(m);
    if (m->eng_wob) { HIPCHK(hipStreamSynchronize(m->ctx->stream)); (void)hipFree(m->eng_wob); m->eng_wob = nullptr; }
    graphs_destroy(m);
    return VOX_OK;
}

extern "C" int32_t vox_model_replicate(const vox_model* src, vox_ctx* dst_ctx, vox_model** out) {
    ARGCHK(src && dst_ctx && out, "null argument");
    if (!src->is_q4 || src->manifest.empty()) return fail(VOX_ERR_UNSUPPORTED, "vox_model_replicate: Q4 (GGUF) models only");
    VOXCHK(ctx_bind(src->ctx)); HIPCHK(hipStreamSynchronize(src->ctx->stream));
    VOXCHK(ctx_bind(dst_ctx));
    ManifestSource ms; ms.m = &src->manifest;
    vox_model* d = nullptr;
    VOXCHK(model_build(dst_ctx, &ms, true, true, &d));
    if (d->arena_primary_bytes != src->arena_primary_bytes || d->arena_bytes != src->arena_bytes) { model_release(d); return fail(VOX_ERR_INVALID, "internal: replica arena layout differs from the source's"); }
    hipError_t e = src->ctx->device == dst_ctx->device ? hipMemcpyAsync(d->arena, src->arena, src->arena_primary_bytes, hipMemcpyDeviceToDevice, dst_ctx->stream)
                                                       : hipMemcpyPeerAsync(d->arena, dst_ctx->device, src->arena, src->ctx->device, src->arena_primary_bytes, dst_ctx->stream);
    if (e == hipSuccess) e = hipStreamSynchronize(dst_ctx->stream);
    if (e != hipSuccess) { model_release(d); return fail(VOX_ERR_HIP, "vox_model_replicate: device copy failed: %s", hipGetErrorString(e)); }
    const int32_t r = vox_model_arena_finalize(d);
    if (r != VOX_OK) { model_release(d); return r; }
    *out = d; return VOX_OK;
}

extern "C" int32_t vox_model_set_t_embed(vox_model* m, const float* t_embed) {
    ARGCHK(m && t_embed, "null argument"); VOXCHK(ctx_bind(m->ctx));
    const vox_model_cfg& c = m->cfg; vox_ctx* cx = m->ctx;
    if (m->t_embed_set && m->t_embed_host.size() == (size_t)c.dec_dim && !std::memcmp(m->t_embed_host.data(), t_embed, (size_t)c.dec_dim * 4)) return VOX_OK;
    DevBuf dt, dh, ones; HIPCHK(dt.alloc((size_t)c.dec_dim * 4)); HIPCHK(dh.alloc((size_t)c.t_cond_dim * 4)); HIPCHK(ones.alloc((size_t)c.dec_dim * 4));
    std::vector<float> one(c.dec_dim, 1.0f);
    HIPCHK(hipMemcpyAsync(dt.p, t_embed, (size_t)c.dec_dim * 4, hipMemcpyHostToDevice, cx->stream));
    HIPCHK(hipMemcpyAsync(ones.p, one.data(), (size_t)c.dec_dim * 4, hipMemcpyHostToDevice, cx->stream));
    for (int i = 0; i < c.dec_layers; i++) {
        VOXCHK(q4_linear_dev(cx, m->dec[i].ada0.w, nullptr, dt.as<float>(), c.dec_dim, 1, dh.as<float>(), c.t_cond_dim, EPI_GELU));
        VOXCHK(q4_linear_dev(cx, m->dec[i].ada2.w, nullptr, dh.as<float>(), c.t_cond_dim, 1, m->dec[i].ada_mul, c.dec_dim, EPI_RESID, ones.as<float>(), c.dec_dim));
    }
    HIPCHK(hipStreamSynchronize(cx->stream));
    m->t_embed_host.assign(t_embed, t_embed + c.dec_dim); m->t_embed_set = true;
    m->pfx.dec_built = false;
    return VOX_OK;
}

static int conv_len(int L) { return (L + 2 - 3) / 2 + 1; }

static int32_t ensure(float** p, size_t* cap, size_t need) {
    if (*cap >= need) return VOX_OK;
    if (*p) HIPCHK(hipFree(*p));
    *p = nullptr; *cap = 0;
    HIPCHK(hipMalloc((void**)p, need * sizeof(float))); *cap = need; return VOX_OK;
}

static int enc_rows(int T) { return conv_len(conv_len(T)); }
static int enc_row_budget(const vox_model* m, const int* T, int n) {
    int mx = 0; for (int i = 0; i < n; i++) mx = std::max(mx, enc_rows(T[i]));
    const int r = m->cfg.reshape_factor; return n == 1 ? mx : (mx + r - 1) / r * r;
}
static size_t conv_scratch_floats(const vox_model* m, int T) {
    const int D = m->cfg.enc_dim, T1 = conv_len(T);
    return std::max((size_t)D * T1, (size_t)(T + 2) * m->cfg.n_mels + (size_t)(T1 + 2) * D) + 64;
}
static int32_t conv_stem_dev(vox_model* m, const float* d_mel, int T, float* c1, float* x) {
    const vox_model_cfg& c = m->cfg; hipStream_t s = m->ctx->stream; const int D = c.enc_dim, T1 = conv_len(T), S = conv_len(T1);
    const bool conv_mfma = m->conv1_g.qs && m->conv2_g.qs && !knob_str("VOX_CONV_VALU");
    if (conv_mfma) {
        const int Cm = c.n_mels;
        float* melT = c1; float* c1T = melT + (size_t)(T + 2) * Cm;
        HIPCHK(hipMemsetAsync(melT, 0, (size_t)Cm * 4, s)); HIPCHK(hipMemsetAsync(melT + (size_t)(T + 1) * Cm, 0, (size_t)Cm * 4, s));
        HIPCHK(hipMemsetAsync(c1T, 0, (size_t)D * 4, s)); HIPCHK(hipMemsetAsync(c1T + (size_t)(T1 + 1) * D, 0, (size_t)D * 4, s));
        HIPCHK(launch_transpose(d_mel, Cm, T, melT + Cm, s));
        { GemmParams g{}; g.w = m->conv1_g; g.x = melT; g.x_stride = 2 * Cm; g.M = T1; g.out = c1T + D; g.out_stride = D; g.bias = m->conv1_b; HIPCHK(launch_dense2_gemm(g, EPI_GELU, s)); }
        { GemmParams g{}; g.w = m->conv2_g; g.x = c1T; g.x_stride = 2 * D; g.M = S; g.out = x; g.out_stride = D; g.bias = m->conv2_b; HIPCHK(launch_dense2_gemm(g, EPI_GELU, s)); }
    } else {
        HIPCHK(launch_conv1d_gelu(d_mel, c.n_mels, T, m->conv1_w, m->conv1_b, D, c1, 0, s));
        HIPCHK(launch_conv1d_gelu(c1, D, T1, m->conv2_w, m->conv2_b, D, x, 1, s));
    }
    return VOX_OK;
}
static int enc_packed_rows_of(const vox_model* m, int T) { const int R = m->cfg.reshape_factor; return std::max((enc_rows(T) + R - 1) / R * R, R * 40); }
static long enc_packed_rows(const vox_model* m, const int* T, int n) { long r = 0; for (int i = 0; i < n; i++) r += enc_packed_rows_of(m, T[i]); return r; }
struct EncForms { long Mtot = 0; int ksp = 0, ksp_wo = 0, fused_rope = 0; };
static int32_t encode_batch_dev(vox_model* m, int n, const float* const* d_mels, const int* T, float* audio_out, int audio_rows, int* S4_out, long* audio_off_out = nullptr,
                                EncForms* forms = nullptr, int prefix_rows = 0) {
    const vox_model_cfg& c = m->cfg; vox_ctx* cx = m->ctx; hipStream_t s = cx->stream;
    const int D = c.enc_dim, H = c.enc_heads, hd = c.enc_head_dim, QD = H * hd, F = c.enc_ffn, R = c.reshape_factor;
    const bool packed = audio_off_out != nullptr;
    ARGCHK(n <= 128, "internal: encoder stack of %d utterances", n);
    const int S_pad = enc_row_budget(m, T, n);
    int T1max = 0; bool any = false;
    std::vector<int> S(n);
    for (int i = 0; i < n; i++) { S[i] = enc_rows(T[i]); S4_out[i] = S[i] / R; T1max = std::max(T1max, conv_len(T[i])); any = any || S4_out[i] > 0; }
    if (!any || S_pad <= 0) return VOX_OK;
    ARGCHK(S_pad <= m->enc_rope_len, "audio too long for the encoder RoPE table (%d > %d positions); chunk it (--max-mel-frames)", S_pad, m->enc_rope_len);
    std::vector<int> roff(n + 1, 0);
    if (packed) for (int i = 0; i < n; i++) roff[i + 1] = roff[i] + enc_packed_rows_of(m, T[i]);
    const int r0 = prefix_rows;
    ARGCHK(r0 == 0 || (n == 1 && !packed && r0 % R == 0 && r0 < S_pad && m->pfx.enc_built && r0 == m->pfx.RC), "internal: encoder prefix of %d rows", r0);
    const int Mfull = packed ? roff[n] : n * S_pad;
// ... 2554 lines not shown
```

### voxtral-mini-realtime-rs_amd/csrc/vox_kernels.h

```cpp
#pragma once
#include <hip/hip_runtime.h>
#include <atomic>
struct DevOnce {
    std::atomic<uint64_t> mask{0};
    bool done(int dev) const { return (mask.load(std::memory_order_acquire) >> (dev & 63)) & 1ull; }
    void set(int dev) { mask.fetch_or(1ull << (dev & 63), std::memory_order_release); }
};
static inline int vox_current_device() { int d = 0; if (hipGetDevice(&d) != hipSuccess) { (void)hipGetLastError(); d = 0; } return d; }
#include <stdint.h>

namespace vox {

struct Q4W {
    const uint4* qs;
    const uint16_t* sc;
    int N, K, nb;
    int fmt;
    const uint4* qt = nullptr; const uint16_t* st = nullptr;
};
enum WFmt { WFMT_Q4_0 = 0, WFMT_BF16 = 1, WFMT_BF16X2 = 2, WFMT_F32 = 3 };

enum Epi { EPI_STORE = 0, EPI_RESID = 1, EPI_SWIGLU = 2, EPI_ROPE_KV = 3, EPI_ARGMAX = 4, EPI_GELU = 5, EPI_SWIGLU_XF = 6, EPI_RESID_XF = 7,
           EPI_ROPE_ROWS = 8 };
enum Pro { PRO_NONE = 0, PRO_RMS = 1, PRO_RMS_MUL = 2,
           PRO_RMS_MUL_SUM = 3 };

struct GemvParams {
    Q4W w;
    const float* x; int x_stride;
    float* out; int out_stride;
    const float* bias;
    const float* resid; int resid_stride;
    const float* gamma; const float* mul; float eps;
    long long* zero_acc; int zero_n;
    const long long* xacc; float* x_out;
    const int* pos_ptr; int pos_off;
    const float* rope_cos; const float* rope_sin; int hd;
    int n_q, n_k;
    float* kcache; float* vcache; int cache_head_stride;
    float* part_val; int* part_idx;
    int tl_slot;
};
hipError_t launch_q4_gemv(const GemvParams& p, int n_rows_x, int pro, int epi, int R, hipStream_t s);
const char* q4_gemv_kernel_name(int K, int pro, int epi, int R);
int q4_gemv_default_R(int N, int K, int epi);
int q4_gemv_grid(int N, int R);
int q4_gemv_nwv(int K, int epi);
int q4_gemv_grid_k(int N, int K, int R, int epi);
int dense_gemv_grid(int N);

struct GemmParams {
    Q4W w;
    const float* x; int x_stride; int M;
    float* out; int out_stride;
    const float* bias;
    const float* resid; int resid_stride;
    const uint4* xf;
    uint16_t* xf_scratch; size_t xf_scratch_bytes;
    const float* ssq_part; int n_part; float norm_eps;
    uint16_t* xf_out; const float* xf_w; const float* xf_w2; float* ssq_out;
    const int* pos; const float* rope_cos; const float* rope_sin; int hd, n_q, n_kv; float* kc; float* vc; long kv_seq_stride; int kv_head_stride;
    const int* kv_row;
    int tl_slot;
    int ksplit;
    float* kz_scratch; size_t kz_scratch_bytes;
    int rope_seq_rows;
    int wide_mt; long xf_gstride , xf_out_gstride , ssq_part_gstride, ssq_out_gstride ;
    int wide_rows;
};
struct WidePlan { int kz, sps, ntw; };
bool q4_wide_plan(const Q4W& w, int mt, int epi, WidePlan* pl);
size_t q4_wide_planes_bytes(const Q4W& w, int mt, const WidePlan& pl);
hipError_t launch_q4_wide(const GemmParams& p, int epi, hipStream_t s);
hipError_t launch_q4_tile_build(Q4W w, uint4* qt, uint16_t* st, hipStream_t s);
hipError_t launch_q4_gemm(const GemmParams& p, int epi, hipStream_t s, bool* fused_rope = nullptr);
hipError_t launch_dense2_gemm(const GemmParams& p, int epi, hipStream_t s);
hipError_t launch_transpose(const float* in, int R, int C, float* out, hipStream_t s);
int q4_skinny_resid_xf_parts(int N);

hipError_t launch_q4_repack(const uint8_t* raw, uint4* qs, uint16_t* sc, int64_t n_blocks, int nb, int row_mul, int row_add, hipStream_t s);
hipError_t launch_q4_dequant(Q4W w, float* out, hipStream_t s);
hipError_t launch_rms_norm(const float* x, int x_stride, int rows, int dim, const float* gamma, const float* mul,
                           float eps, float* out, int out_stride, hipStream_t s);
hipError_t launch_rms_norm_sumk(float* x, int x_stride, int rows, int dim, const float* part, size_t part_stride, int ksplit, const float* gamma, float eps, float* out, int out_stride, hipStream_t s);
int q4_skinny_mt2_plan(const Q4W& w, int M);
hipError_t launch_xf_rows(const float* x, int x_stride, int M, int K, uint16_t* xf, hipStream_t s);
hipError_t launch_q4_skinny_mt2_planes(const GemmParams& p, int KZ, hipStream_t s);
hipError_t launch_splitk_finish_resid(const float* planes, int KZ, int M, int N, float* x, int x_stride, hipStream_t s);
hipError_t launch_splitk_finish_swiglu_xf(const float* planes, int KZ, int M, int N, const float* bias, uint16_t* xf, hipStream_t s);
hipError_t launch_splitk_finish_rope_kv(const float* planes, int KZ, int M, int N, float* q_out, int q_stride, int n_q, int n_kv, int hd, int pos_off,
                                        const float* cos_t, const float* sin_t, float* kc, float* vc, int head_stride, hipStream_t s);
hipError_t launch_rms_norm_xf_sumk(float* x, int x_stride, int rows, int dim, const float* planes, int kz, const float* gamma, const float* mul, float eps, uint16_t* xf, hipStream_t s);
hipError_t launch_rms_norm_xf(const float* x, int x_stride, int rows, int dim, const float* gamma, const float* mul,
                              float eps, uint16_t* xf, hipStream_t s);
hipError_t launch_rope(float* buf, int M, int stride, int n_rot, int hd, int pos_off, const float* cos_t,
                       const float* sin_t, hipStream_t s, int seq_rows = 0, const int* row_pos = nullptr);
hipError_t launch_kv_store(const float* buf, int M, int stride, int k_col, int n_kv, int hd, int pos_off,
                           float* kcache, float* vcache, int cache_head_stride, hipStream_t s, int seq_rows = 0, long kv_seq_stride = 0);

struct AttnParams {
    const float* q; int q_stride;
    const float* k; const float* v;
    int kv_row_stride, kv_head_stride;
    float* out; int out_stride;
    int M, kv_len, n_heads, n_kv_heads, offset, window;
    const int* pos_ptr;
    int pos_per_seq; int q_seq_stride, out_seq_stride; long kv_seq_stride;
    const int* kv_row;
    const int* seq_len;
    const int* seq_row_off;
    uint16_t* out_xf_tiles; long out_xf_tile_stride;
    uint16_t* out_xf;
    long out_xf_gstride;
    int prefer_gqa;
    int no_xcd_remap;
    int tl_slot;
    int spec_zero;
    int spec_rows;
    const float* prefix_k; const float* prefix_v; int prefix_len, prefix_row_stride, prefix_head_stride;
};
hipError_t launch_attn_prefill(const AttnParams& p, int hd, hipStream_t s, int n_seq = 1);
bool attn_prefill_prefix_ok(const AttnParams& p, int hd, int n_seq);
bool attn_prefill_small_ok(const AttnParams& p, int hd, int n_seq);
hipError_t launch_attn_decode(const AttnParams& p, int hd, int max_seq, hipStream_t s, int n_seq = 1);
bool attn_wo_supported(const AttnParams& p, const Q4W& wo, int hd, int max_seq);
hipError_t launch_attn_wo(const AttnParams& p, const Q4W& wo, long long* acc, int max_seq, hipStream_t s);
enum AttnForm { ATTN_FORM_PREFILL_SMALL, ATTN_FORM_PREFILL_MFMA, ATTN_FORM_PREFILL_F32, ATTN_FORM_DECODE, ATTN_FORM_DECODE_SPEC, ATTN_FORM_DECODE_GQA, ATTN_FORM_WO,
                ATTN_FORM_ENGINE, ATTN_FORM_STREAM_RING, ATTN_FORM_COUNT };
void attn_form_note(AttnForm f);
void attn_form_counts(unsigned long long out[ATTN_FORM_COUNT]);
enum GemmForm { GEMM_FORM_GEMV_R1, GEMM_FORM_GEMV_R2, GEMM_FORM_GEMV_R4, GEMM_FORM_DENSE_GEMV, GEMM_FORM_SKINNY, GEMM_FORM_SKINNY_MT, GEMM_FORM_SKINNY_MT2, GEMM_FORM_XF_ROWS,
                GEMM_FORM_SPLITK_FINISH, GEMM_FORM_TILE_11, GEMM_FORM_TILE_12, GEMM_FORM_TILE_21, GEMM_FORM_TILE_22, GEMM_FORM_TILE_21_TB, GEMM_FORM_TILE_22_TB, GEMM_FORM_K32,
                GEMM_FORM_BIG, GEMM_FORM_BIG_ROPE, GEMM_FORM_DENSE2, GEMM_FORM_WIDE, GEMM_FORM_COUNT };
void gemm_form_counts(unsigned long long out[GEMM_FORM_COUNT]);

hipError_t launch_conv1d_gelu(const float* in, int Cin, int L, const float* w, const float* b, int Cout, float* out,
                              int out_token_major, hipStream_t s);

struct MelTables { const float* window; const float* cos_t; const float* sin_t; const float* fb; const int* fb_lo; const int* fb_hi; };
hipError_t launch_mel(const float* audio, long n, long left, long right, const float* scale_ptr, MelTables t,
                      float* out, int T, int transposed, hipStream_t s);
hipError_t launch_resample_matrix(const double* H, int new_len, int fft_in, int fft_out, float* At, hipStream_t s);
hipError_t launch_resample(const float* x, long n_in, const float* At, int fft_in, int fft_out, int delay, float* out, long n_out, hipStream_t s);
hipError_t launch_absmax(const float* x, long n, float target_peak, float* scale_out, hipStream_t s);
hipError_t launch_absmax_group(const float* x, long n, unsigned* group_max_cell, hipStream_t s);
hipError_t launch_group_scale(const unsigned* group_max, const int* unit_group, int n, float target, float* unit_scale, hipStream_t s);

hipError_t launch_embed(Q4W tok, const int* ids, int n, const float* audio, int D, const int* pos_ptr, int id_off,
                        int a_off, float* out, hipStream_t s);
hipError_t launch_argmax_final(const float* part_val, const int* part_idx, int n_parts, int* tokens, int* pos_ptr,
                               int tok_off, int inc, hipStream_t s);
hipError_t launch_argmax_embed(const float* part_val, const int* part_idx, int n_parts, int* tokens, int* pos_ptr, Q4W tok,
                               const float* audio, int D, float* h, hipStream_t s);
hipError_t launch_rope_kv_batch(float* qkv, int n, int stride, int n_q, int n_kv, int hd, const int* pos, const float* cos_t, const float* sin_t,
                                float* kcache, float* vcache, long seq_stride, int head_stride, hipStream_t s);
hipError_t launch_argmax_embed_batch(const float* logits, int n, int vocab, int* tokens, int tok_stride, int* pos, const int* seq_len, Q4W tok,
                                     const float* audio, long audio_seq_stride, int D, float* h, hipStream_t s,
                                     uint16_t* xf = nullptr, const float* xf_w = nullptr, float* ssq_out = nullptr,
                                     long xf_group_stride = 0, int ssq_group_stride = 0,
                                     const long* audio_off = nullptr);
struct SlotStepParams {
    const float* logits; int vocab;
    int* tokens; int tok_stride; const int* clip_len;
    int* slot_clip; int* slot_qpos; const int* queue; int q_stride;
    int* pos; int* kv_row; int n_clips; int first_pos;
    Q4W tok; const float* audio; const long* audio_off; int D;
    const float* h0;
    float* h;
    uint16_t* xf; const float* xf_w; float* ssq_out; long xf_group_stride; int ssq_group_stride;
    int init;
};
hipError_t launch_argmax_embed_slots(const SlotStepParams& p, int n_slots, hipStream_t s);
struct BatchTapParams {
    const float* logits; int vocab;
    const int* slot_clip; int clip0; const int* pos; const int* seq_len;
    const int* clip_unit; int n_clips;
    float* out; int* rows; int n_units, max_rows, first_pos;
};
hipError_t launch_batch_tap(const BatchTapParams& p, int n_rows, hipStream_t s);
hipError_t launch_occupy(int workgroups, int micros, hipStream_t s);
hipError_t launch_add_rows(const float* a, const float* b, float* out, long n, hipStream_t s);
hipError_t launch_gelu(float* x, long n, hipStream_t s);
hipError_t launch_argmax_rows(const float* x, int rows, int V, int* out, hipStream_t s);

struct EngLayerTab { const float* attn_norm; const float* ffn_norm; const float* ada_mul; float* kc; float* vc; };
struct EngParams {
    const unsigned char* stream; size_t cu_stride;
    const EngLayerTab* layers; int n_layers;
    const float* h_in;
    const float* final_norm;
    const int* pos_ptr; int pos_off;
    const float* rope_cos; const float* rope_sin;
    int max_seq, window; float eps;
    unsigned long long *H0, *H1, *G, *PW, *A, *P2;
    unsigned long long *SS0, *SS1;
    unsigned long long* XC;
    unsigned* serial; unsigned* err;
    float* part_val; int* part_idx;
    int* tokens; int* pos_rw; const uint4* tok_qs; const uint16_t* tok_sc; int tok_nb; const float* audio;
    float* logits_out;
    int vocab;
    unsigned long long* tl; int tl_layer;
    int flags;
    int ag_delay_ticks;
    int pace_ticks;
};
bool eng_geometry_ok(int D, int n_heads, int n_kv, int hd, int ffn, int vocab, int max_seq);
size_t eng_stream_bytes(int n_layers, int vocab);
size_t eng_state_bytes();
hipError_t launch_eng_pack(const Q4W& w, int op, int layer, int n_layers, unsigned char* stream, int vocab, hipStream_t s);
void eng_state_carve(unsigned char* state, EngParams* p);
hipError_t launch_decode_engine(const EngParams& p, hipStream_t s);
hipError_t launch_eng_hidden(const EngParams& p, float* out, hipStream_t s);
hipError_t eng_occupancy(int* blocks_per_cu);
int eng_lds_bytes();

// ... 68 lines not shown
```

### voxtral-mini-realtime-rs_amd/csrc/vox_kernels.hip

```cpp
#include "vox_kernels.h"

#include <hip/hip_fp16.h>

#include <unistd.h>

#include <algorithm>
#include <atomic>
#include <cstdio>
#include <cstdlib>
#include <cstring>
#include <string>
#include <mutex>
#include <unordered_map>

namespace vox {

static int g_tl_next = -1, g_tl_slots = 0;
#ifdef VOX_TIMELINE
__device__ unsigned long long* g_tl_buf = nullptr;
__device__ int g_tl_waves = 0;
__device__ __forceinline__ void tl_stamp(int slot, int wave_global, int k) {
    if (slot >= 0 && (wave_global & 3) == 0 && (threadIdx.x & 63) == 0 && g_tl_buf && wave_global < g_tl_waves)
        g_tl_buf[((size_t)slot * g_tl_waves + wave_global) * 4 + k] = wall_clock64();
}
// ... 721 lines not shown
    xa = *reinterpret_cast<const float4*>(xrow + 32 * (B_) + xoff_a);        \
    xb = *reinterpret_cast<const float4*>(xrow + 32 * (B_) + xoff_b);                                               \
    if (FMT == WFMT_Q4_0) { wd = wq[(size_t)(B_) * 4]; wsc = ws[(B_)]; }    \
    else { wdv = wd16[(size_t)(B_) * 4]; }
#define VOX_STAGE(BUF_)                                                                            \
    { uint4 hi_, lo_; split_bf16x8(xa, xb, hi_, lo_); lds[(BUF_)][0][slot] = hi_; lds[(BUF_)][1][slot] = lo_; }
    float4 xa, xb; uint32_t wd = 0; uint16_t wsc = 0; uint4 wdv = make_uint4(0, 0, 0, 0);
    VOX_GLOAD(0)
    VOX_STAGE(0)
    uint32_t cur_wd = wd; uint16_t cur_sc = wsc; uint4 cur_wdv = wdv;
    { const int b1 = min(1, nb - 1); VOX_GLOAD(b1) }
    __syncthreads();
    for (int b = 0; b < nb; b++) {
        const int buf = b & 1;
        const float4 sxa = xa, sxb = xb; const uint32_t swd = wd; const uint16_t ssc = wsc; const uint4 swdv = wdv;
        { const int b2 = min(b + 2, nb - 1); VOX_GLOAD(b2) }
        const bf16x8 bw = as_bf16x8(FMT == WFMT_Q4_0 ? q4_dword_to_bf16x8(cur_wd) : cur_wdv);
        const float d = FMT == WFMT_Q4_0 ? f16_bits_to_f32(cur_sc) : 1.0f;
#pragma unroll
        for (int mt = 0; mt < 4; mt++) {
            const bf16x8 ah = as_bf16x8(lds[buf][0][mt * 64 + lane]);
            const bf16x8 al = as_bf16x8(lds[buf][1][mt * 64 + lane]);
            f32x4 t = __builtin_amdgcn_mfma_f32_16x16x32_bf16(ah, bw, (f32x4){0.f, 0.f, 0.f, 0.f}, 0, 0, 0);
            t = __builtin_amdgcn_mfma_f32_16x16x32_bf16(al, bw, t, 0, 0, 0);
            acc[mt][0] = fmaf(d, t[0], acc[mt][0]); acc[mt][1] = fmaf(d, t[1], acc[mt][1]);
            acc[mt][2] = fmaf(d, t[2], acc[mt][2]); acc[mt][3] = fmaf(d, t[3], acc[mt][3]);
        }
        if (b + 1 < nb) {
            uint4 hi_, lo_; split_bf16x8(sxa, sxb, hi_, lo_); lds[buf ^ 1][0][slot] = hi_; lds[buf ^ 1][1][slot] = lo_;
            cur_wd = swd; cur_sc = ssc; cur_wdv = swdv;
        }
        __syncthreads();
    }
#undef VOX_GLOAD
#undef VOX_STAGE
    const float bias = (p.bias && wrow_ok) ? p.bias[wn] : 0.f;
#pragma unroll
    for (int mt = 0; mt < 4; mt++)
#pragma unroll
        for (int r = 0; r < 4; r++) {
            const int m = m0 + mt * 16 + 4 * (lane >> 4) + r;
            float v = acc[mt][r] + bias;
            if (EPI == EPI_SWIGLU) {
                const float other = dpp_mov<0xB1>(v);
                if (m < M && wrow_ok && !(wn & 1)) p.out[(size_t)m * p.out_stride + (wn >> 1)] = silu_f(v) * other;
            } else if (m < M && wrow_ok) {
                if (EPI == EPI_RESID) v = v + p.resid[(size_t)m * p.resid_stride + wn];
                if (EPI == EPI_GELU) v = gelu_f(v);
                p.out[(size_t)m * p.out_stride + wn] = v;
            }
        }
}

template <int MT, int NT, int EPI, int FMT, int TB = 0>
__global__ __launch_bounds__(256) __attribute__((amdgpu_waves_per_eu(2))) void q4_gemm_kernel(const GemmParams p) {
    extern __shared__ __attribute__((aligned(16))) uint4 glds[];
    constexpr int PLANE = 4 * MT * 64, BUF = 2 * PLANE;
    const int nb = p.w.nb, N = p.w.N, M = p.M, nq = nb >> 2;
    const int tid = threadIdx.x, lane = tid & 63, wave = tid >> 6;
    const int m0 = blockIdx.y * (16 * MT), n0 = blockIdx.x * (64 * NT);
    const int KSP = p.ksplit > 1 ? p.ksplit : 1, kz = blockIdx.z;
    const int qb = (int)((long)nq * kz / KSP), qe = (int)((long)nq * (kz + 1) / KSP);
    const float* xrow[MT]; int slot[MT], xo_a[MT], xo_b[MT];
#pragma unroll
    for (int i = 0; i < MT; i++) {
        const int f = tid + 256 * i, sm = f >> 4, j = (f >> 2) & 3, g = f & 3;
        xrow[i] = p.x + (size_t)min(m0 + sm, M - 1) * p.x_stride;
        slot[i] = (j * MT + (sm >> 4)) * 64 + g * 16 + ((sm & 15) ^ (4 * j + g));
        xo_a[i] = 32 * j + (FMT == WFMT_Q4_0 ? 4 * g : 8 * g); xo_b[i] = 32 * j + (FMT == WFMT_Q4_0 ? 16 + 4 * g : 8 * g + 4);
    }
    const int wg = lane >> 4;
    int rdl[4];
#pragma unroll
    for (int j = 0; j < 4; j++) rdl[j] = (lane & 48) | ((lane & 15) ^ (4 * j + wg));
    const uint32_t* wq[NT]; const uint16_t* ws[NT]; const uint4* wd16[NT]; const uint4* wqt[NT]; int wn[NT]; bool wok[NT];
#pragma unroll
    for (int t = 0; t < NT; t++) {
        wn[t] = n0 + (wave * NT + t) * 16 + (lane & 15); wok[t] = wn[t] < N;
        const size_t row = (size_t)min(wn[t], N - 1);
        wq[t] = reinterpret_cast<const uint32_t*>(p.w.qs) + row * nb * 4 + wg;
        ws[t] = FMT == WFMT_Q4_0 ? p.w.sc + row * nb : nullptr;
        wd16[t] = p.w.qs + row * nb * 4 + wg;
        const size_t T = (size_t)min((n0 >> 4) + wave * NT + t, ((N + 15) >> 4) - 1);
        wqt[t] = TB ? p.w.qt + T * nq * 64 + lane : nullptr;
    }
    f32x4 acc[NT][MT];
#pragma unroll
    for (int t = 0; t < NT; t++)
#pragma unroll
        for (int i = 0; i < MT; i++) acc[t][i] = (f32x4){0.f, 0.f, 0.f, 0.f};

    float4 xa[MT], xb[MT];
    uint32_t wd[NT][4]; uint2 wsc[NT]; uint4 wdv[NT][4];
#define VOX_GLOAD(Q_)                                                                                          \
    _Pragma("unroll") for (int i = 0; i < MT; i++) {                                                           \
        xa[i] = *reinterpret_cast<const float4*>(xrow[i] + 128 * (Q_) + xo_a[i]);                              \
        xb[i] = *reinterpret_cast<const float4*>(xrow[i] + 128 * (Q_) + xo_b[i]);                              \
    }                                                                                                          \
    _Pragma("unroll") for (int t = 0; t < NT; t++) {                                                           \
        if (FMT == WFMT_Q4_0) {                                                                                \
            if (TB) { const uint4 w4 = ld_nt_u4(wqt[t] + (size_t)64 * (Q_)); wd[t][0] = w4.x; wd[t][1] = w4.y; wd[t][2] = w4.z; wd[t][3] = w4.w; } \
            else { _Pragma("unroll") for (int j = 0; j < 4; j++) wd[t][j] = wq[t][(size_t)(4 * (Q_) + j) * 4]; } \
            wsc[t] = *reinterpret_cast<const uint2*>(ws[t] + 4 * (Q_));                                        \
        } else {                                                                                               \
            _Pragma("unroll") for (int j = 0; j < 4; j++) wdv[t][j] = wd16[t][(size_t)(4 * (Q_) + j) * 4];     \
        }                                                                                                      \
    }
#define VOX_STAGE(BUF_)                                                                                        \
    _Pragma("unroll") for (int i = 0; i < MT; i++) {                                                           \
        uint4 hi_, lo_; split_bf16x8(sxa[i], sxb[i], hi_, lo_);                                                \
        glds[(BUF_) * BUF + slot[i]] = hi_; glds[(BUF_) * BUF + PLANE + slot[i]] = lo_;                        \
    }
    VOX_GLOAD(qb)
    float4 sxa[MT], sxb[MT];
#pragma unroll
    for (int i = 0; i < MT; i++) { sxa[i] = xa[i]; sxb[i] = xb[i]; }
    VOX_STAGE(0)
    uint32_t cwd[NT][4]; uint2 csc[NT]; uint4 cwdv[NT][4];
#pragma unroll
    for (int t = 0; t < NT; t++) { csc[t] = wsc[t];
#pragma unroll
        for (int j = 0; j < 4; j++) { cwd[t][j] = wd[t][j]; cwdv[t][j] = wdv[t][j]; } }
    { const int q1 = min(qb + 1, qe - 1); VOX_GLOAD(q1) }
    __syncthreads();
    for (int q = qb; q < qe; q++) {
        const int buf = (q - qb) & 1;
#pragma unroll
        for (int i = 0; i < MT; i++) { sxa[i] = xa[i]; sxb[i] = xb[i]; }
        uint32_t nwd[NT][4]; uint2 nsc[NT]; uint4 nwdv[NT][4];
#pragma unroll
        for (int t = 0; t < NT; t++) { nsc[t] = wsc[t];
#pragma unroll
            for (int j = 0; j < 4; j++) { nwd[t][j] = wd[t][j]; nwdv[t][j] = wdv[t][j]; } }
        { const int q2 = min(q + 2, qe - 1); VOX_GLOAD(q2) }
#pragma unroll
        for (int j = 0; j < 4; j++) {
#pragma unroll
            for (int t = 0; t < NT; t++) {
                const bf16x8 bw = as_bf16x8(FMT == WFMT_Q4_0 ? q4_dword_to_bf16x8(cwd[t][j]) : cwdv[t][j]);
                float d = 1.0f;
                if (FMT == WFMT_Q4_0) {
                    const uint32_t pr = (j & 2) ? csc[t].y : csc[t].x;
                    d = f16_bits_to_f32((uint16_t)((j & 1) ? (pr >> 16) : (pr & 0xFFFFu)));
                }
#pragma unroll
                for (int i = 0; i < MT; i++) {
                    const bf16x8 ah = as_bf16x8(glds[buf * BUF + (j * MT + i) * 64 + rdl[j]]);
                    const bf16x8 al = as_bf16x8(glds[buf * BUF + PLANE + (j * MT + i) * 64 + rdl[j]]);
                    f32x4 tt = __builtin_amdgcn_mfma_f32_16x16x32_bf16(ah, bw, (f32x4){0.f, 0.f, 0.f, 0.f}, 0, 0, 0);
                    tt = __builtin_amdgcn_mfma_f32_16x16x32_bf16(al, bw, tt, 0, 0, 0);
                    acc[t][i][0] = fmaf(d, tt[0], acc[t][i][0]); acc[t][i][1] = fmaf(d, tt[1], acc[t][i][1]);
                    acc[t][i][2] = fmaf(d, tt[2], acc[t][i][2]); acc[t][i][3] = fmaf(d, tt[3], acc[t][i][3]);
                }
            }
        }
        if (q + 1 < qe) {
            VOX_STAGE(buf ^ 1)
#pragma unroll
            for (int t = 0; t < NT; t++) { csc[t] = nsc[t];
#pragma unroll
                for (int j = 0; j < 4; j++) { cwd[t][j] = nwd[t][j]; cwdv[t][j] = nwdv[t][j]; } }
        }
        __syncthreads();
    }
#undef VOX_GLOAD
#undef VOX_STAGE
#pragma unroll
    for (int t = 0; t < NT; t++) {
        const float bias = (p.bias && wok[t] && kz == 0) ? p.bias[wn[t]] : 0.f;
#pragma unroll
        for (int i = 0; i < MT; i++)
#pragma unroll
            for (int r = 0; r < 4; r++) {
                const int m = m0 + i * 16 + 4 * (lane >> 4) + r;
                float v = acc[t][i][r] + bias;
                if (EPI == EPI_SWIGLU) {
                    const float other = dpp_mov<0xB1>(v);
                    if (m < M && wok[t] && !(wn[t] & 1)) p.out[(size_t)m * p.out_stride + (wn[t] >> 1)] = silu_f(v) * other;
                } else if (m < M && wok[t]) {
                    if (EPI == EPI_RESID) v = v + p.resid[(size_t)m * p.resid_stride + wn[t]];
                    if (EPI == EPI_GELU) v = gelu_f(v);
                    (p.out + (size_t)kz * p.M * p.out_stride)[(size_t)m * p.out_stride + wn[t]] = v;
                }
            }
    }
}

__global__ void q4_tile_build_kernel(Q4W w, uint4* __restrict__ qt, uint16_t* __restrict__ st, int n_tiles) {
    const int nq = w.nb >> 2;
    const long total = (long)n_tiles * nq * 64;
    for (long i = (long)blockIdx.x * blockDim.x + threadIdx.x; i < total; i += (long)gridDim.x * blockDim.x) {
        const int lane = (int)(i & 63); const long tq = i >> 6; const int q = (int)(tq % nq), T = (int)(tq / nq);
        const int g = lane >> 4, n = T * 16 + (lane & 15);
        uint32_t d[4] = {0x88888888u, 0x88888888u, 0x88888888u, 0x88888888u};
        if (n < w.N) {
            const uint32_t* src = reinterpret_cast<const uint32_t*>(w.qs) + ((size_t)n * w.nb + 4 * q) * 4 + g;
#pragma unroll
            for (int j = 0; j < 4; j++) d[j] = src[j * 4];
        }
        qt[i] = make_uint4(d[0], d[1], d[2], d[3]);
        if (g == 0) {
#pragma unroll
            for (int j = 0; j < 4; j++) st[(tq * 16 + (lane & 15)) * 4 + j] = n < w.N ? w.sc[(size_t)n * w.nb + 4 * q + j] : (uint16_t)0;
        }
    }
}
hipError_t launch_q4_tile_build(Q4W w, uint4* qt, uint16_t* st, hipStream_t s) {
    if (w.nb % 4) return hipErrorInvalidValue;
    const int n_tiles = (w.N + 15) / 16;
    q4_tile_build_kernel<<<dim3(2048), dim3(256), 0, s>>>(w, qt, st, n_tiles);
    return hipGetLastError();
}

template <int NTW, int EPI, int TILED, int XIN, int PRO, int STEPS = 0>
__global__ __launch_bounds__(NTW == 3 ? 256 : 512, NTW == 3 ? 3 : 1) void q4_skinny_kernel(const GemmParams p) {
    extern __shared__ __attribute__((aligned(16))) float sred[];
    __shared__ float s_rstd[16]; __shared__ float s_pp[32 * 16];
    const int nb = p.w.nb, N = p.w.N, M = p.M, nq = nb >> 2;
    const int tid = threadIdx.x, lane = tid & 63, wave = tid >> 6, KS = blockDim.x >> 6;
    const int g = lane >> 4, li = lane & 15;
    const int nbase = blockIdx.x * (16 * NTW);
    const int tlw = wave == 0 ? (int)blockIdx.x * 4 : 1; (void)tlw;
    VOX_TL(p.tl_slot, tlw, 0);
    const float* xrow = p.x + (size_t)min(li, M - 1) * p.x_stride;
    const uint4* wq[NTW]; const uint16_t* ws[NTW];
    const int n_tiles = (N + 15) >> 4;
#pragma unroll
    for (int t = 0; t < NTW; t++) {
        if (TILED) {
            const size_t T = (size_t)min(blockIdx.x * NTW + t, n_tiles - 1);
            wq[t] = p.w.qt + T * nq * 64 + lane; ws[t] = p.w.st + (T * nq * 16 + li) * 4;
        } else {
            const size_t row = (size_t)min(nbase + t * 16 + li, N - 1);
            wq[t] = p.w.qs + row * nb + g; ws[t] = p.w.sc + row * nb;
        }
    }
    f32x4 acc[NTW];
#pragma unroll
    for (int t = 0; t < NTW; t++) acc[t] = (f32x4){0.f, 0.f, 0.f, 0.f};
    uint4 wv[NTW], wvn[NTW]; uint2 sv[NTW], svn[NTW]; float4 xa[4], xb[4];
    const uint4* xfh = p.xf + lane; const uint4* xfl = p.xf + (size_t)nq * 256 + lane;
#define VOX_WLOAD(WV_, SV_, Q_)                                                                            \
    _Pragma("unroll") for (int t = 0; t < NTW; t++) {                                                      \
        WV_[t] = ld_nt_u4(wq[t] + (TILED ? 64 : 4) * (Q_)); SV_[t] = *reinterpret_cast<const uint2*>(ws[t] + (TILED ? 64 : 4) * (Q_)); }
#define VOX_XLOAD(Q_)                                                                                      \
    _Pragma("unroll") for (int j = 0; j < 4; j++) {                                                        \
        if (XIN) {                                                                                         \
            xa[j] = *reinterpret_cast<const float4*>(xfh + ((Q_) * 4 + j) * 64);                           \
            xb[j] = *reinterpret_cast<const float4*>(xfl + ((Q_) * 4 + j) * 64);                           \
        } else {                                                                                           \
            xa[j] = *reinterpret_cast<const float4*>(xrow + 128 * (Q_) + 32 * j + 4 * g);                  \
            xb[j] = *reinterpret_cast<const float4*>(xrow + 128 * (Q_) + 32 * j + 16 + 4 * g); } }
#define VOX_SSTEP(WV_, SV_, XA_, XB_)                                                                      \
    {                                                                                                      \
        const bf16x8 m136 = as_bf16x8(make_uint4(0xC308C308u, 0xC308C308u, 0xC308C308u, 0xC308C308u));     \
        uint32_t dw[NTW][4];                                                                               \
        _Pragma("unroll") for (int t = 0; t < NTW; t++) {                                                  \
            dw[t][0] = WV_[t].x; dw[t][1] = WV_[t].y; dw[t][2] = WV_[t].z; dw[t][3] = WV_[t].w;            \
            if (!TILED) {                            \
                auto s01 = __builtin_amdgcn_permlane16_swap(WV_[t].x, WV_[t].y, false, false);             \
                auto s23 = __builtin_amdgcn_permlane16_swap(WV_[t].z, WV_[t].w, false, false);             \
                auto u02 = __builtin_amdgcn_permlane32_swap(s01[0], s23[0], false, false);                 \
                auto u13 = __builtin_amdgcn_permlane32_swap(s01[1], s23[1], false, false);                 \
                dw[t][0] = u02[0]; dw[t][1] = u13[0]; dw[t][2] = u02[1]; dw[t][3] = u13[1];                \
            }                                                                                              \
        }                                                                                                  \
               \
        _Pragma("unroll") for (int j = 0; j < 4; j++) {                                                    \
            uint4 ah, al;                                                                                  \
            if (XIN) {                                                                                     \
                ah = make_uint4(__float_as_uint(XA_[j].x), __float_as_uint(XA_[j].y), __float_as_uint(XA_[j].z), __float_as_uint(XA_[j].w)); \
                al = make_uint4(__float_as_uint(XB_[j].x), __float_as_uint(XB_[j].y), __float_as_uint(XB_[j].z), __float_as_uint(XB_[j].w)); \
            } else {                                                                                       \
                split_pair(XA_[j].x, XA_[j].z, ah.x, al.x); split_pair(XB_[j].x, XB_[j].z, ah.y, al.y);    \
                split_pair(XA_[j].y, XA_[j].w, ah.z, al.z); split_pair(XB_[j].y, XB_[j].w, ah.w, al.w);    \
            }                                                                                              \
            const f32x4 sx = __builtin_amdgcn_mfma_f32_16x16x32_bf16(as_bf16x8(ah), m136, (f32x4){0.f, 0.f, 0.f, 0.f}, 0, 0, 0); \
            const f32x4 cs = __builtin_amdgcn_mfma_f32_16x16x32_bf16(as_bf16x8(al), m136, sx, 0, 0, 0);    \
            _Pragma("unroll") for (int t = 0; t < NTW; t++) {                                              \
                const bf16x8 bw = as_bf16x8(q4_dword_to_bf16x8_biased(dw[t][j]));                          \
                const uint32_t sc2 = (j >> 1) ? SV_[t].y : SV_[t].x;                                       \
                const float d = f16_bits_to_f32((uint16_t)((j & 1) ? (sc2 >> 16) : (sc2 & 0xFFFFu)));      \
                f32x4 tt = __builtin_amdgcn_mfma_f32_16x16x32_bf16(as_bf16x8(ah), bw, cs, 0, 0, 0);        \
                tt = __builtin_amdgcn_mfma_f32_16x16x32_bf16(as_bf16x8(al), bw, tt, 0, 0, 0);              \
                acc[t] = __builtin_elementwise_fma((f32x4){d, d, d, d}, tt, acc[t]);                        \
            }                                                                                              \
        }                                                                                                  \
    }
// ... 1077 lines not shown
    return hipGetLastError();
}
__global__ void transpose_kernel(const float* __restrict__ in, int R, int C, float* __restrict__ out) {
    __shared__ float tile[32][33];
    const int c0 = blockIdx.x * 32, r0 = blockIdx.y * 32, tx = threadIdx.x & 31, ty = threadIdx.x >> 5;
    for (int k = ty; k < 32; k += 8) { const int r = r0 + k, c = c0 + tx; tile[k][tx] = (r < R && c < C) ? in[(size_t)r * C + c] : 0.f; }
    __syncthreads();
    for (int k = ty; k < 32; k += 8) { const int c = c0 + k, r = r0 + tx; if (c < C && r < R) out[(size_t)c * R + r] = tile[tx][k]; }
}
hipError_t launch_transpose(const float* in, int R, int C, float* out, hipStream_t s) {
    transpose_kernel<<<dim3((C + 31) / 32, (R + 31) / 32), dim3(256), 0, s>>>(in, R, C, out);
    return hipGetLastError();
}

template <int NTW, int TILED>
static hipError_t skinny_launch_n(const GemmParams& p, int epi, int ks, hipStream_t s) {
    dim3 grid((p.w.N + 16 * NTW - 1) / (16 * NTW));
    const size_t lds = (size_t)ks * NTW * 64 * 4 * sizeof(float);
    if (p.xf) {
        if (!TILED) return hipErrorInvalidValue;
        const bool pro = p.ssq_part != nullptr;
        if (pro && (p.n_part < 1 || p.n_part > 12 * (64 * ks / 16))) return hipErrorInvalidValue;
        const int nq = p.w.nb / 4, per = nq % ks == 0 ? nq / ks : 0;
        if (per) {
#define VOX_ST(N_, E_, P_, S_) if (NTW == N_ && epi == E_ && (int)pro == P_ && per == S_) { \
            if (E_ == EPI_RESID_XF && (!p.xf_out || !p.xf_w || !p.ssq_out)) return hipErrorInvalidValue; \
            q4_skinny_kernel<N_, E_, 1, 1, P_, S_><<<grid, dim3(64 * ks), lds, s>>>(p); return hipGetLastError(); }
            VOX_ST(2, EPI_ROPE_KV, 1, 3) VOX_ST(2, EPI_SWIGLU_XF, 1, 6) VOX_ST(1, EPI_SWIGLU_XF, 1, 6) VOX_ST(1, EPI_RESID_XF, 0, 4) VOX_ST(4, EPI_SWIGLU_XF, 1, 6) VOX_ST(1, EPI_RESID_XF, 0, 9) VOX_ST(4, EPI_STORE, 1, 6)
#undef VOX_ST
        }
        if (epi == EPI_RESID_XF) {
            if (NTW != 1 || pro || !p.xf_out || !p.xf_w || !p.ssq_out) return hipErrorInvalidValue;
            q4_skinny_kernel<1, EPI_RESID_XF, 1, 1, 0><<<grid, dim3(64 * ks), lds, s>>>(p);
        } else if (pro) {
            switch (epi) {
            case EPI_STORE: q4_skinny_kernel<NTW, EPI_STORE, 1, 1, 1><<<grid, dim3(64 * ks), lds, s>>>(p); break;
            case EPI_ROPE_KV: q4_skinny_kernel<NTW, EPI_ROPE_KV, 1, 1, 1><<<grid, dim3(64 * ks), lds, s>>>(p); break;
            case EPI_SWIGLU_XF: q4_skinny_kernel<NTW, EPI_SWIGLU_XF, 1, 1, 1><<<grid, dim3(64 * ks), lds, s>>>(p); break;
            default: return hipErrorInvalidValue;
            }
        } else {
            switch (epi) {
            case EPI_STORE: q4_skinny_kernel<NTW, EPI_STORE, 1, 1, 0><<<grid, dim3(64 * ks), lds, s>>>(p); break;
            case EPI_RESID: q4_skinny_kernel<NTW, EPI_RESID, 1, 1, 0><<<grid, dim3(64 * ks), lds, s>>>(p); break;
            case EPI_SWIGLU_XF: q4_skinny_kernel<NTW, EPI_SWIGLU_XF, 1, 1, 0><<<grid, dim3(64 * ks), lds, s>>>(p); break;
            default: return hipErrorInvalidValue;
            }
        }
        return hipGetLastError();
    }
    switch (epi) {
    case EPI_STORE: q4_skinny_kernel<NTW, EPI_STORE, TILED, 0, 0><<<grid, dim3(64 * ks), lds, s>>>(p); break;
    case EPI_RESID: q4_skinny_kernel<NTW, EPI_RESID, TILED, 0, 0><<<grid, dim3(64 * ks), lds, s>>>(p); break;
    case EPI_GELU: q4_skinny_kernel<NTW, EPI_GELU, TILED, 0, 0><<<grid, dim3(64 * ks), lds, s>>>(p); break;
    case EPI_SWIGLU: q4_skinny_kernel<NTW, EPI_SWIGLU, TILED, 0, 0><<<grid, dim3(64 * ks), lds, s>>>(p); break;
    default: return hipErrorInvalidValue;
    }
    return hipGetLastError();
}
int q4_skinny_resid_xf_parts(int N) { return (N + 15) / 16; }
static hipError_t launch_q4_skinny(const GemmParams& p_in, int epi, hipStream_t s) {
    GemmParams p = p_in; p.tl_slot = tl_take_slot(2, epi, p.w.N, p.w.K);
    const int nq = p.w.nb / 4, tiles = (p.w.N + 15) / 16;
    int ntw = tiles >= 4 * 192 ? 4 : (tiles >= 2 * 192 ? 2 : 1);
    int ks = nq >= 4 ? 4 : (nq >= 2 ? 2 : 1);
    if (tiles / ntw < 256 && nq >= 16) ks = 8;
    if (epi == EPI_RESID_XF) ntw = 1;
    const bool tiled = p.w.qt && p.w.st;
    hipError_t e;
    if (ntw == 4) e = tiled ? skinny_launch_n<4, 1>(p, epi, ks, s) : skinny_launch_n<4, 0>(p, epi, ks, s);
    else if (ntw == 2) e = tiled ? skinny_launch_n<2, 1>(p, epi, ks, s) : skinny_launch_n<2, 0>(p, epi, ks, s);
    else e = tiled ? skinny_launch_n<1, 1>(p, epi, ks, s) : skinny_launch_n<1, 0>(p, epi, ks, s);
    if (e == hipSuccess) gemm_form_note(GEMM_FORM_SKINNY);
    return e;
}

template <int MT, int NT, int FMT, int TB = 0>
static hipError_t gemm_launch_mn(const GemmParams& p, int epi, hipStream_t s) {
    if (p.ksplit > 1 && (epi != EPI_STORE || p.ksplit > p.w.nb / 4)) return hipErrorInvalidValue;
    dim3 grid((p.w.N + 64 * NT - 1) / (64 * NT), (p.M + 16 * MT - 1) / (16 * MT), p.ksplit > 1 ? p.ksplit : 1);
    const size_t lds = (size_t)2 * 2 * 4 * MT * 64 * sizeof(uint4);
#define VOX_E(E_) case E_: { auto kern = q4_gemm_kernel<MT, NT, E_, FMT, TB>; static DevOnce done;      \
        hipError_t e = ensure_dyn_lds(kern, lds, &done); if (e != hipSuccess) return e;                       \
        gemm_form_note(TB ? (NT == 2 ? GEMM_FORM_TILE_22_TB : GEMM_FORM_TILE_21_TB) : MT == 1 ? (NT == 2 ? GEMM_FORM_TILE_12 : GEMM_FORM_TILE_11) : (NT == 2 ? GEMM_FORM_TILE_22 : GEMM_FORM_TILE_21)); \
        kern<<<grid, dim3(256), lds, s>>>(p); break; }
    switch (epi) { VOX_E(EPI_STORE) VOX_E(EPI_RESID) VOX_E(EPI_GELU) VOX_E(EPI_SWIGLU) default: return hipErrorInvalidValue; }
#undef VOX_E
    return hipGetLastError();
}
template <int FMT>
static hipError_t gemm_launch_f(const GemmParams& p, int epi, hipStream_t s) {
    if (p.w.nb % 4) {
        dim3 grid((p.w.N + 63) / 64, (p.M + 63) / 64);
        if (epi != EPI_STORE && epi != EPI_RESID && epi != EPI_GELU && epi != EPI_SWIGLU) return hipErrorInvalidValue;
        gemm_form_note(GEMM_FORM_K32);
        switch (epi) {
        case EPI_STORE: q4_gemm_k32_kernel<EPI_STORE, FMT><<<grid, dim3(256), 0, s>>>(p); break;
        case EPI_RESID: q4_gemm_k32_kernel<EPI_RESID, FMT><<<grid, dim3(256), 0, s>>>(p); break;
        case EPI_GELU: q4_gemm_k32_kernel<EPI_GELU, FMT><<<grid, dim3(256), 0, s>>>(p); break;
        case EPI_SWIGLU: q4_gemm_k32_kernel<EPI_SWIGLU, FMT><<<grid, dim3(256), 0, s>>>(p); break;
        default: return hipErrorInvalidValue;
        }
        return hipGetLastError();
    }
    const int mt = p.M <= 48 ? 1 : 2;
    int nt = 2;
    auto wgs = [&](int mt_, int nt_) { return (long)((p.w.N + 64 * nt_ - 1) / (64 * nt_)) * ((p.M + 16 * mt_ - 1) / (16 * mt_)); };
    if (wgs(mt, 2) < 256) nt = 1;
    if (FMT == WFMT_Q4_0 && p.w.qt && p.w.st && mt == 2) {
        if (wgs(2, 2) >= 128) nt = 2;
        return nt == 2 ? gemm_launch_mn<2, 2, WFMT_Q4_0, 1>(p, epi, s) : gemm_launch_mn<2, 1, WFMT_Q4_0, 1>(p, epi, s);
    }
#define VOX_MN(M_, N_) if (mt == M_ && nt == N_) return gemm_launch_mn<M_, N_, FMT>(p, epi, s)
    VOX_MN(1, 1); VOX_MN(1, 2); VOX_MN(2, 1); VOX_MN(2, 2);
#undef VOX_MN
    return hipErrorInvalidValue;
}
hipError_t launch_rope(float* buf, int M, int stride, int n_rot, int hd, int pos_off, const float* cos_t, const float* sin_t, hipStream_t s, int seq_rows, const int* row_pos);
static hipError_t launch_q4_gemm_epi(const GemmParams& p, int epi, hipStream_t s, bool* fused_rope);
hipError_t launch_q4_gemm(const GemmParams& p, int epi, hipStream_t s, bool* fused_rope) {
    if (fused_rope) *fused_rope = false;
    if (epi != EPI_ROPE_ROWS) return launch_q4_gemm_epi(p, epi, s, nullptr);
    if (!p.rope_cos || !p.rope_sin || p.hd <= 0 || p.n_q <= 0 || p.n_q > p.w.N || p.n_q % 2) return hipErrorInvalidValue;
    bool fused = false;
    hipError_t e = launch_q4_gemm_epi(p, EPI_ROPE_ROWS, s, &fused);
    if (fused_rope) *fused_rope = fused;
    if (e != hipSuccess || fused) return e;
    return launch_rope(p.out, p.M, p.out_stride, p.n_q, p.hd, 0, p.rope_cos, p.rope_sin, s, p.rope_seq_rows, p.pos);
}
static hipError_t launch_q4_gemm_epi(const GemmParams& p, int epi_in, hipStream_t s, bool* fused_rope) {
    int epi = epi_in == EPI_ROPE_ROWS ? EPI_STORE : epi_in;
    if (p.w.K % 32 || p.M <= 0) return hipErrorInvalidValue;
    if (p.ksplit > 1 && (p.M <= 48 || p.xf || p.w.nb % 4 || p.w.fmt == WFMT_F32)) return hipErrorInvalidValue;
    if (p.w.fmt == WFMT_F32) {
        if (p.xf) return hipErrorInvalidValue;
        GemmParams v = p; v.w.fmt = WFMT_BF16X2; v.w.qt = nullptr; v.w.st = nullptr;
        return launch_dense2_gemm(v, epi, s);
    }
    if (p.xf && p.M > 16) return (p.M <= 48 && p.w.fmt == WFMT_Q4_0 && p.w.nb % 4 == 0 && p.w.qt && p.w.st && (epi == EPI_STORE || epi == EPI_RESID || epi == EPI_GELU || epi == EPI_SWIGLU))
                                     ? launch_q4_skinny_mt(p, epi, s) : hipErrorInvalidValue;
    if (p.xf) return (p.M <= 16 && p.w.fmt == WFMT_Q4_0 && p.w.nb % 4 == 0 && p.w.qt) ? launch_q4_skinny(p, epi, s) : hipErrorInvalidValue;
    if (p.M <= 16 && p.w.fmt == WFMT_Q4_0 && p.w.nb % 4 == 0 && !env_int("VOX_NO_SKINNY")) return launch_q4_skinny(p, epi, s);
    if (p.M > 16 && p.M <= 48 && p.w.fmt == WFMT_Q4_0 && p.w.qt && p.w.st && p.w.nb % 4 == 0 && (p.x_stride % 4) == 0 && (epi == EPI_STORE || epi == EPI_RESID || epi == EPI_GELU || epi == EPI_SWIGLU) &&
        !env_int("VOX_NO_SKINNY_MT")) {
        return launch_q4_skinny_mt(p, epi, s);
    }
    if (p.w.fmt == WFMT_Q4_0 && p.w.qt && p.w.st && p.w.nb % 4 == 0 && (p.x_stride % 4) == 0) {
        const int big = env_int("VOX_GEMM_BIG");
        const long wg14 = (long)((p.w.N + 255) / 256) * ((p.M + 63) / 64);
        const int big_min = 200;
        const bool fits32 = ((size_t)(p.M - 1) * p.x_stride + (size_t)p.w.K) * 4 < 0xFFFFFFF0ull && (size_t)((p.w.N + 15) / 16) * (p.w.nb / 4) * 1024 < 0xFFFFFFF0ull;
        if (p.ksplit <= 1 && fits32 && p.w.N % 256 == 0 && (big == 1 || (big == 0 && wg14 >= big_min))) {
            if (epi_in == EPI_ROPE_ROWS && wg14 >= 1024 && (p.hd & (p.hd - 1)) == 0 && !knob_str("VOX_NO_ROPE_FUSE")) { if (fused_rope) *fused_rope = true; return gemm_big_launch<1, 4>(p, EPI_ROPE_ROWS, s); }
            return gemm_big_launch<1, 4>(p, epi, s);
        }
    }
    return p.w.fmt == WFMT_BF16 ? gemm_launch_f<WFMT_BF16>(p, epi, s) : gemm_launch_f<WFMT_Q4_0>(p, epi, s);
}

__global__ __launch_bounds__(256) void rms_norm_kernel(const float* __restrict__ x, int x_stride, int rows, int dim,
                                                       const float* __restrict__ gamma, const float* __restrict__ mul,
                                                       float eps, float* __restrict__ out, int out_stride) {
    const int row = min(blockIdx.x * 4 + (threadIdx.x >> 6), rows - 1), lane = threadIdx.x & 63;
    const float4* xr = reinterpret_cast<const float4*>(x + (size_t)row * x_stride);
    const int n4 = dim >> 2;
    float4 v[16];
    float ss = 0.f;
#pragma unroll
    for (int i = 0; i < 16; i++) {
        const int c = lane + 64 * i;
        v[i] = xr[min(c, n4 - 1)];
        if (c < n4) ss += (v[i].x * v[i].x + v[i].y * v[i].y) + (v[i].z * v[i].z + v[i].w * v[i].w);
    }
    for (int c = lane + 1024; c < n4; c += 64) { const float4 t = xr[c]; ss += (t.x * t.x + t.y * t.y) + (t.z * t.z + t.w * t.w); }
    ss = wave_sum(ss);
    const float rms = sqrtf(ss / (float)dim + eps);
    float4* o = reinterpret_cast<float4*>(out + (size_t)row * out_stride);
    const float4* g4 = reinterpret_cast<const float4*>(gamma);
    const float4* m4 = reinterpret_cast<const float4*>(mul);
#define VOX_RMS_OUT(T_, C_)                                                                                     \
    { float4 t = (T_); const float4 gm = g4[C_];                                                                \
      t.x = (t.x / rms) * gm.x; t.y = (t.y / rms) * gm.y; t.z = (t.z / rms) * gm.z; t.w = (t.w / rms) * gm.w;   \
      if (mul) { const float4 mm = m4[C_]; t.x *= mm.x; t.y *= mm.y; t.z *= mm.z; t.w *= mm.w; }               \
      o[C_] = t; }
#pragma unroll
    for (int i = 0; i < 16; i++) {
        const int c = lane + 64 * i;
        if (c < n4) VOX_RMS_OUT(v[i], c)
    }
    for (int c = lane + 1024; c < n4; c += 64) VOX_RMS_OUT(xr[c], c)
#undef VOX_RMS_OUT
}
__global__ __launch_bounds__(256) void rms_norm_row_kernel(const float* __restrict__ x, int x_stride, int dim, const float* __restrict__ gamma,
// ... 1595 lines not shown
```

### voxtral-mini-realtime-rs_amd/gguf.py

```python
from __future__ import annotations

import ctypes as C
import weakref

import numpy as np

from . import _lib
from ._lib import check, lib, VoxError

F32, F16, Q4_0 = 0, 1, 2


def _f32(a):
    return np.ascontiguousarray(a, dtype=np.float32)


def _ptr(a):
    return a.ctypes.data_as(C.c_void_p)


class Context:

    def __init__(self, device: int = 0):
        self.h = C.c_void_p()
# ... 78 lines not shown
        return cls(path)

    @classmethod
    def from_bytes(cls, data):
        r = cls(); r._keep = np.frombuffer(data, dtype=np.uint8)
        check(lib().vox_gguf_open_memory(r._keep.ctypes.data, r._keep.size, C.byref(r.h)))
        return r

    @classmethod
    def from_shards(cls, shards):
        arrs = [np.frombuffer(s, dtype=np.uint8) for s in shards]; n = len(arrs)
        ptrs = (C.c_void_p * n)(*[a.ctypes.data for a in arrs]); sizes = (C.c_size_t * n)(*[a.size for a in arrs])
        r = cls(); check(lib().vox_gguf_open_shards(ptrs, sizes, n, C.byref(r.h)))
        return r

    def version(self):
        v = C.c_uint32(); check(lib().vox_gguf_version(self.h, C.byref(v))); return v.value

    def tensor_count(self):
        v = C.c_uint64(); check(lib().vox_gguf_tensor_count(self.h, C.byref(v))); return v.value

    def tensor_names(self):
        out = []
        for i in range(self.tensor_count()):
            s = C.c_char_p(); check(lib().vox_gguf_tensor_name(self.h, i, C.byref(s))); out.append(s.value.decode())
        return out

    def tensor_info(self, name):
        dims = (C.c_uint64 * 4)(); nd = C.c_uint32(); dt = C.c_uint32(); nb = C.c_uint64()
        r = lib().vox_gguf_tensor_info(self.h, name.encode(), C.byref(dims), C.byref(nd), C.byref(dt), C.byref(nb))
        if r == 4:
            return None
        check(r)
        return GgufTensorInfo(name, [int(dims[i]) for i in range(nd.value)], dt.value, nb.value)

    def tensor_data(self, name):
        info = self.tensor_info(name)
        if info is None:
            raise VoxError(4, f"Tensor '{name}' not found in GGUF")
        out = np.empty(info.byte_size(), dtype=np.uint8)
        check(lib().vox_gguf_tensor_data(self.h, name.encode(), _ptr(out), out.size))
        return out

    def close(self):
        if self.h:
            lib().vox_gguf_close(self.h); self.h = None

    def __del__(self):
        try:
            self.close()
        except Exception:
            pass


class Q4Tensor:

    def __init__(self, ctx, h, shape):
        self.ctx, self.h, self._shape = ctx, h, shape

    @classmethod
    def from_q4_bytes(cls, raw_bytes, shape, ctx: Context):
        raw = np.ascontiguousarray(np.frombuffer(raw_bytes, dtype=np.uint8) if not isinstance(raw_bytes, np.ndarray) else raw_bytes, dtype=np.uint8)
        n, k = shape; h = C.c_void_p()
        check(lib().vox_q4_tensor_from_bytes(ctx.h, _ptr(raw), raw.size, n, k, C.byref(h)))
        return cls(ctx, h, [n, k])

    @classmethod
    def from_f32(cls, w, ctx: Context, other=None):
        w = _f32(w); n, k = w.shape; h = C.c_void_p()
        o = None if other is None else _f32(other)
        check(lib().vox_dense_tensor_from_f32(ctx.h, _ptr(w), None if o is None else _ptr(o), n, k, C.byref(h)))
        return cls(ctx, h, [n if o is None else 2 * n, k])

    def shape(self):
        return list(self._shape)

    def num_blocks(self):
        v = C.c_int64(); check(lib().vox_q4_tensor_num_blocks(self.h, C.byref(v))); return v.value

    def dequantize(self):
        out = np.empty(self._shape, dtype=np.float32)
        check(lib().vox_q4_tensor_dequantize(self.ctx.h, self.h, _ptr(out)))
        return out

    def close(self):
        if self.h:
            lib().vox_q4_tensor_free(self.h); self.h = None

    def __del__(self):
        try:
            self.close()
        except Exception:
            pass


def q4_matmul(x, weights: Q4Tensor):
    x = _f32(x)
    if x.ndim != 3:
        raise VoxError(1, f"q4_matmul expects a 3-D input, got {x.ndim}-D")
    b, m, k = x.shape
    n, kw = weights.shape()
    if k != kw:
        raise VoxError(1, f"q4_matmul: input K={k} != weight K={kw}")
    out = np.empty((b, m, n), dtype=np.float32)
    check(lib().vox_q4_matmul(weights.ctx.h, weights.h, _ptr(x), b, m, _ptr(out), 0))
    return out


def linear_forward(weights: Q4Tensor, x, bias=None, epilogue=0):
    x = _f32(x)
    if x.ndim != 3:
        raise VoxError(1, f"linear_forward expects a 3-D input, got {x.ndim}-D")
    b, m, k = x.shape; n, kw = weights.shape()
    if k != kw:
        raise VoxError(1, f"linear_forward: input K={k} != weight K={kw}")
    if bias is not None and np.size(bias) != n:
        raise VoxError(1, f"linear_forward: bias has {np.size(bias)} elements, weight N={n}")
    out = np.empty((b, m, n // 2 if epilogue == 2 else n), dtype=np.float32)
    bb = None if bias is None else _f32(bias)
    check(lib().vox_linear_forward_ex(weights.ctx.h, weights.h, None if bb is None else _ptr(bb), _ptr(x), b, m, _ptr(out), epilogue, 0))
    return out


def conv_downsample(ctx, x, w1, b1, w2, b2):
    x, w1, b1, w2, b2 = (_f32(a) for a in (x, w1, b1, w2, b2))
    c_, l_ = x.shape; o_ = w1.shape[0]; l2 = ((l_ + 1) // 2 + 1) // 2
    out = np.empty((o_, l2), dtype=np.float32)
    check(lib().vox_conv_downsample(ctx.h, _ptr(x), c_, l_, _ptr(w1), _ptr(b1), _ptr(w2), _ptr(b2), o_, _ptr(out)))
    return out


def attention(ctx, q, k, v, n_heads, n_kv_heads, offset=0, window=-1):
    q, k, v = _f32(q), _f32(k), _f32(v)
    if q.ndim != 2 or k.ndim != 2 or k.shape != v.shape or q.shape[1] % n_heads:
        raise VoxError(1, "attention: bad shapes")
    hd = q.shape[1] // n_heads
    if k.shape[1] != n_kv_heads * hd:
        raise VoxError(1, "attention: k/v width != n_kv_heads*head_dim")
    out = np.empty_like(q)
    check(lib().vox_attention(ctx.h, _ptr(q), _ptr(k), _ptr(v), q.shape[0], k.shape[0], n_heads, n_kv_heads, hd, offset, window, _ptr(out), 0))
    return out


class Q4Linear:

    def __init__(self, weights: Q4Tensor, bias=None):
        self.weights = weights
        self.bias = None if bias is None else _f32(bias)

    @classmethod
    def new(cls, weights, bias=None):
        return cls(weights, bias)

    def forward(self, x):
        x = _f32(x); b, m, k = x.shape; n = self.weights.shape()[0]
        out = np.empty((b, m, n), dtype=np.float32)
        check(lib().vox_q4_linear_forward(self.weights.ctx.h, self.weights.h, None if self.bias is None else _ptr(self.bias),
                                          _ptr(x), b, m, _ptr(out), 0))
        return out


class LayerCaches:

    def __init__(self, model, max_seq):
        self.model = model; self.h = C.c_void_p()
        check(lib().vox_decoder_cache_create(model.h, max_seq, C.byref(self.h)))
# ... 127 lines not shown

    def finish(self) -> np.ndarray:
        return self._ids(lambda o, c, n: lib().vox_stream_finish(self.h, o, c, n), 0, True)

    def reset(self):
        check(lib().vox_stream_reset(self.h))

    def info(self):
        v = (C.c_int64 * 8)(); check(lib().vox_stream_info(self.h, v))
        return dict(zip(("samples", "positions", "ids", "encoder_position", "ring_rows", "bytes", "engine_steps", "operator_steps"), (int(x) for x in v)))

    def tap_arm(self, max_rows):
        check(lib().vox_debug_stream_tap_arm(self.h, int(max_rows))); self._tap_max = int(max_rows)

    def tap_fetch(self):
        buf = np.zeros((self._tap_max, self.model.config.vocab), dtype=np.float32); rows = C.c_int32()
        check(lib().vox_debug_stream_tap_fetch(self.h, _ptr(buf), C.byref(rows)))
        if rows.value > self._tap_max:
            raise VoxError(1, f"stream tap: {rows.value} rows for a tap of {self._tap_max}")
        return buf[:rows.value].copy()

    def close(self):
        if self.h:
            lib().vox_stream_free(self.h); self.h = None

    def __del__(self):
        try:
            self.close()
        except Exception:
            pass


class Q4VoxtralModel:

    def __init__(self, ctx, h):
        self.ctx, self.h = ctx, h
        self._caches = weakref.WeakSet()
        self.config = _lib.ModelCfg(); check(lib().vox_model_config(h, C.byref(self.config)))

    def decoder(self):
        return Q4LanguageModel(self)

    def create_decoder_cache_preallocated(self, max_seq):
        return LayerCaches(self, max_seq)

    def generate_step_with_cache(self, token_ids, t_embed, caches):
        ids = np.ascontiguousarray(token_ids, dtype=np.int32).reshape(-1)
        out = np.empty((ids.size, self.config.vocab), dtype=np.float32)
        check(lib().vox_generate_step_with_cache(self.h, _ptr(ids), ids.size, _ptr(_f32(t_embed).reshape(-1)), caches.h, _ptr(out)))
        return out

    def _mel2(self, mel):
        mel = _f32(mel); return mel.reshape(mel.shape[-2], mel.shape[-1])

    def forward(self, mel, t_embed):
        mel = self._mel2(mel); T = mel.shape[1]; cap = T // 16 + 2
        out = np.empty((cap, self.config.vocab), dtype=np.float32); S = C.c_int32()
        check(lib().vox_forward(self.h, _ptr(mel), T, _ptr(_f32(t_embed).reshape(-1)), _ptr(out), cap, C.byref(S), 0))
        return out[:S.value][None].copy()

    def forward_streaming(self, mel, token_ids, t_embed):
        mel = self._mel2(mel); T = mel.shape[1]; cap = T // 16 + 2
        ids = np.ascontiguousarray(token_ids, dtype=np.int32).reshape(-1)
        out = np.empty((cap, self.config.vocab), dtype=np.float32); S = C.c_int32()
        check(lib().vox_forward_streaming(self.h, _ptr(mel), T, _ptr(ids), ids.size, _ptr(_f32(t_embed).reshape(-1)), _ptr(out), cap, C.byref(S), 0))
        return out[:S.value][None].copy()

    def forward_with_cache(self, mel, t_embed, encoder_cache, decoder_cache):
        mel = self._mel2(mel); T = mel.shape[1]; cap = T // 16 + 2
        out = np.empty((cap, self.config.vocab), dtype=np.float32); S = C.c_int32()
        check(lib().vox_forward_with_cache(self.h, _ptr(mel), T, _ptr(_f32(t_embed).reshape(-1)), encoder_cache.h, decoder_cache.h, _ptr(out), cap, C.byref(S), 0))
        return out[:S.value][None].copy()

    def set_decode_engine(self, on: bool) -> bool:
        a = C.c_int32(); check(lib().vox_model_set_decode_engine(self.h, 1 if on else 0, C.byref(a))); return bool(a.value)

    def set_prefix_cache(self, on=None) -> bool:
        a = C.c_int32(); check(lib().vox_model_set_prefix_cache(self.h, -1 if on is None else (1 if on else 0), C.byref(a))); return bool(a.value)

    def prefix_info(self):
        v = (C.c_int32 * 4)(); check(lib().vox_model_prefix_info(self.h, v)); return {"built": bool(v[0]), "encoder_rows": v[1], "decoder_positions": v[2], "bytes": v[3]}

    def memory(self):
        v = (C.c_uint64 * 4)(); check(lib().vox_model_memory(self.h, v)); return {"arena": v[0], "arena_primary": v[1], "engine_stream": v[2], "engine_state": v[3]}

    def set_batch_engine(self, on=None):
        a = C.c_int32(); n = C.c_uint64()
        check(lib().vox_model_set_batch_engine(self.h, -1 if on is None else (1 if on else 0), C.byref(a), C.byref(n))); return bool(a.value), int(n.value)

    def weight_bytes(self):
        v = C.c_uint64(); check(lib().vox_model_weight_bytes(self.h, C.byref(v))); return v.value

    def arena(self):
        p = C.c_void_p(); n = C.c_uint64(); check(lib().vox_model_arena(self.h, C.byref(p), C.byref(n)))
        return p.value, n.value

    def replicate(self, dst_ctx):
        h = C.c_void_p(); check(lib().vox_model_replicate(self.h, dst_ctx.h, C.byref(h)))
        return type(self)(dst_ctx, h)

    def set_sessions(self, sessions: int):
        check(lib().vox_model_set_sessions(self.h, int(sessions)))

    def arena_finalize(self):
        check(lib().vox_model_arena_finalize(self.h))

    def encode_audio(self, mel):
        mel = _f32(mel); mel = mel.reshape(mel.shape[-2], mel.shape[-1]); T = mel.shape[1]
        cap = T // 16 + 2
        out = np.empty((cap, self.config.dec_dim), dtype=np.float32); S = C.c_int32()
        check(lib().vox_encode_audio(self.h, _ptr(mel), T, _ptr(out), cap, C.byref(S), 0))
        return out[:S.value].reshape(1, S.value, self.config.dec_dim).copy()

    def debug_encode_batch(self, mels, layout):
        arrs = [_f32(x) for x in mels]; arrs = [np.ascontiguousarray(a.reshape(a.shape[-2], a.shape[-1])) for a in arrs]; n = len(arrs)
        Ts = [a.shape[1] for a in arrs]
        cap = sum(T // 16 + 2 for T in Ts)
        D = self.config.dec_dim
        out = np.zeros((cap, D), dtype=np.float32); rows = (C.c_int32 * max(n, 1))(); rep = (C.c_int64 * 4)()
        ptrs = (C.c_void_p * max(n, 1))(*[a.ctypes.data for a in arrs])
        check(lib().vox_debug_encode_batch(self.h, n, ptrs, (C.c_int32 * max(n, 1))(*Ts), layout, _ptr(out), cap, rows, rep))
        res, o = [], 0
        for i in range(n):
            res.append(out[o:o + rows[i]].copy()); o += rows[i]
        return res, {"Mtot": rep[0], "ksp": rep[1], "ksp_wo": rep[2], "fused_rope": rep[3]}

    def create_encoder_cache(self, capacity_rows=0):
        return EncoderCaches(self, capacity_rows)

    def encode_audio_with_cache(self, mel, encoder_cache):
        mel = _f32(mel); mel = mel.reshape(mel.shape[-2], mel.shape[-1]); T = mel.shape[1]
        cap = T // 16 + 2
        out = np.empty((cap, self.config.dec_dim), dtype=np.float32); S = C.c_int32()
        check(lib().vox_encode_audio_with_cache(self.h, _ptr(mel), T, encoder_cache.h, _ptr(out), cap, C.byref(S), 0))
        return out[:S.value].reshape(1, S.value, self.config.dec_dim).copy()

    def transcribe_streaming(self, mel, t_embed, return_logits=False):
        mel = _f32(mel); mel = mel.reshape(mel.shape[-2], mel.shape[-1]); T = mel.shape[1]
        cap = T // 16 + 2
        ids = np.zeros(cap, dtype=np.int32); n = C.c_int32()
        t = _f32(t_embed).reshape(-1)
        lg = np.empty((cap, self.config.vocab), dtype=np.float32) if return_logits else None
        check(lib().vox_transcribe_streaming(self.h, _ptr(mel), T, _ptr(t), _ptr(ids), cap, C.byref(n),
                                             None if lg is None else _ptr(lg), 0))
        if return_logits:
            return ids[:n.value].copy(), lg[:n.value].copy()
        return ids[:n.value].copy()

    def transcribe_audio(self, samples, t_embed, device_ptr=None, n_samples=None):
        t = _f32(t_embed).reshape(-1)
        if device_ptr is None:
            x = _f32(samples); n_samples = x.size; ptr = _ptr(x); kind = 0
        else:
            ptr = C.c_void_p(device_ptr); kind = 1
        cap = n_samples // 1280 + 128
        ids = np.zeros(cap, dtype=np.int32); n = C.c_int32()
        check(lib().vox_transcribe_audio(self.h, ptr, n_samples, _ptr(t), _ptr(ids), cap, C.byref(n), kind))
        return ids[:n.value].copy()

    def create_stream(self, t_embed, gain=1.0, enc_capacity_rows=0, max_positions=0) -> LiveStream:
        return LiveStream(self, t_embed, gain, enc_capacity_rows, max_positions)

    def transcribe_batch(self, samples_list, t_embed, device_ptrs=None, n_samples=None, norm_group=None, tap_units=None):
        t = _f32(t_embed).reshape(-1)
        if device_ptrs is None:
            arrs = [_f32(x) for x in samples_list]; n = len(arrs)
            ptrs = (C.c_void_p * n)(*[a.ctypes.data for a in arrs]); lens = (C.c_size_t * n)(*[a.size for a in arrs]); kind = 0
# ... 80 lines not shown
```

Measured before the change: 1496.

## Pre-expand encoder Q4 weights to tile-ordered bf16 for the MT=2 GEMM

Adds a pre-dequantized, tile-ordered bf16 copy of selected encoder weights (wqkv, wo, w2), on by default through VOX_ENC_EXPAND. The MT=2 tiled Q4 GEMM gains a variant that loads bf16x8 directly, skipping the per-dword Q4-to-bf16 unpack. This cuts ALU work in encoder GEMMs, but each expanded weight reads about four times the bytes and uses extra arena memory. It mostly targets encoder prefill; decode token throughput is affected only indirectly.

```diff
diff --git a/include/voxtral_hip.h b/include/voxtral_hip.h
--- a/include/voxtral_hip.h
+++ b/include/voxtral_hip.h
@@ -120,6 +120,7 @@
 int32_t vox_model_arena_finalize(vox_model* m);
 int32_t vox_model_replicate(const vox_model* src, vox_ctx* dst_ctx, vox_model** out);
 int32_t vox_model_memory(const vox_model* m, uint64_t out[4]);
+int32_t vox_model_memory_ex(const vox_model* m, uint64_t* out, int32_t cap);
 
 int32_t vox_model_set_t_embed(vox_model* m, const float* t_embed_host);
 int32_t vox_model_set_decode_engine(vox_model* m, int32_t on, int32_t* active_or_null);
@@ -178,6 +179,7 @@
 int32_t vox_debug_attn_launches(uint64_t* out, int32_t cap);
 int32_t vox_debug_gemm_launches(uint64_t* out, int32_t cap);
 int32_t vox_debug_occupy(vox_ctx* ctx, int32_t workgroups, int32_t micros);
+int32_t vox_debug_q4_expand(vox_q4* q, int32_t on);
 
 int32_t vox_bench_decode_gemv(vox_model* m, int32_t which, int32_t iters, double* avg_us, double* bytes_per_launch,
                               const char** kernel_name);
diff --git a/voxtral-mini-realtime-rs_amd/_lib.py b/voxtral-mini-realtime-rs_amd/_lib.py
--- a/voxtral-mini-realtime-rs_amd/_lib.py
+++ b/voxtral-mini-realtime-rs_amd/_lib.py
@@ -102,6 +102,8 @@
     "vox_model_prefix_info": (i32, [vp, P(i32 * 4)]),
     "vox_debug_occupy": (i32, [vp, i32, i32]),
     "vox_model_memory": (i32, [vp, P(C.c_uint64)]),
+    "vox_model_memory_ex": (i32, [vp, P(C.c_uint64), i32]),
+    "vox_debug_q4_expand": (i32, [vp, i32]),
     "vox_model_set_batch_engine": (i32, [vp, i32, P(i32), P(C.c_uint64)]),
     "vox_model_arena_finalize": (i32, [vp]),
     "vox_model_replicate": (i32, [vp, vp, P(vp)]),
diff --git a/voxtral-mini-realtime-rs_amd/csrc/vox_api.cpp b/voxtral-mini-realtime-rs_amd/csrc/vox_api.cpp
--- a/voxtral-mini-realtime-rs_amd/csrc/vox_api.cpp
+++ b/voxtral-mini-realtime-rs_amd/csrc/vox_api.cpp
@@ -519,7 +519,7 @@
     std::memcpy(dst, g->data(t), t->nbytes); return VOX_OK;
 }
 
-struct vox_q4 { vox_ctx* ctx; Q4W w; void* qs_mem; void* sc_mem; void* qt_mem = nullptr; void* st_mem = nullptr; };
+struct vox_q4 { vox_ctx* ctx; Q4W w; void* qs_mem; void* sc_mem; void* qt_mem = nullptr; void* st_mem = nullptr; void* xt_mem = nullptr; };
 
 static int32_t upload_repack(vox_ctx* c, const uint8_t* raw, int64_t n_blocks, int nb, uint4* qs, uint16_t* sc, int row_mul, int row_add,
                              void* staging, size_t staging_cap) {
@@ -560,7 +560,19 @@
 extern "C" int32_t vox_q4_tensor_free(vox_q4* q) {
     if (!q) return VOX_OK;
     (void)hipSetDevice(q->ctx->device); (void)hipStreamSynchronize(q->ctx->stream);
-    (void)hipFree(q->qs_mem); (void)hipFree(q->sc_mem); (void)hipFree(q->qt_mem); (void)hipFree(q->st_mem); delete q; return VOX_OK;
+    (void)hipFree(q->qs_mem); (void)hipFree(q->sc_mem); (void)hipFree(q->qt_mem); (void)hipFree(q->st_mem); (void)hipFree(q->xt_mem); delete q; return VOX_OK;
+}
+extern "C" int32_t vox_debug_q4_expand(vox_q4* q, int32_t on) {
+    ARGCHK(q, "null argument"); VOXCHK(ctx_bind(q->ctx)); HIPCHK(hipStreamSynchronize(q->ctx->stream));
+    if (!on) { q->w.xt = nullptr; if (q->xt_mem) { (void)hipFree(q->xt_mem); q->xt_mem = nullptr; } return VOX_OK; }
+    if (q->w.xt) return VOX_OK;
+    if (q->w.fmt != WFMT_Q4_0 || q->w.nb % 4 || !q->w.qt || !q->w.st) return fail(VOX_ERR_UNSUPPORTED, "vox_debug_q4_expand: the tensor has no tile-ordered copy (K %% 128 != 0)");
+    const size_t n_tiles = (size_t)(q->w.N + 15) / 16, nq = (size_t)q->w.nb / 4;
+    HIPCHK(hipMalloc(&q->xt_mem, n_tiles * nq * 256 * sizeof(uint4)));
+    hipError_t e = launch_q4_expand_build(q->w, (uint4*)q->xt_mem, q->ctx->stream);
+    if (e == hipSuccess) e = hipStreamSynchronize(q->ctx->stream);
+    if (e != hipSuccess) { (void)hipFree(q->xt_mem); q->xt_mem = nullptr; return fail(VOX_ERR_HIP, "vox_debug_q4_expand: %s", hipGetErrorString(e)); }
+    q->w.xt = (const uint4*)q->xt_mem; return VOX_OK;
 }
 extern "C" int32_t vox_q4_tensor_dequantize(vox_ctx* c, const vox_q4* q, float* out) {
     ARGCHK(c && q && out, "null argument"); VOXCHK(ctx_bind(c));
@@ -744,6 +756,7 @@
     std::map<std::string, TensorMeta> manifest; bool is_q4 = false;
     uint8_t* arena = nullptr; uint64_t arena_bytes = 0, arena_primary_bytes = 0;
     std::vector<Q4W*> tiled;
+    std::vector<Q4W*> expanded; uint64_t expand_bytes = 0; bool enc_expand = false;
     const float *conv1_w = nullptr, *conv1_b = nullptr, *conv2_w = nullptr, *conv2_b = nullptr, *enc_norm = nullptr, *dec_norm = nullptr;
     Q4W conv1_g{}, conv2_g{};
     const float *enc_cos = nullptr, *enc_sin = nullptr, *dec_cos = nullptr, *dec_sin = nullptr;
@@ -957,7 +970,7 @@
         }
         return true;
     }
-    bool lin(const std::vector<std::string>& parts, bool interleave, Lin* L, bool require_q4, bool tile = true) {
+    bool lin(const std::vector<std::string>& parts, bool interleave, Lin* L, bool require_q4, bool tile = true, bool expand = false) {
         int64_t K = -1, Ntot = 0; std::vector<TensorView> ts; int kind = -1;
         for (auto& n : parts) {
             TensorView t; if (!need(n, &t)) return false;
@@ -993,6 +1006,13 @@
                     if (launch_q4_tile_build(L->w, qt, st, m->ctx->stream) != hipSuccess || hipStreamSynchronize(m->ctx->stream) != hipSuccess)
                         return setfail("q4_tile_build failed");
                 }
+                if (expand && m->enc_expand) {
+                    uint4* xt = ar2.take<uint4>(n_tiles * nq * 256);
+                    L->w.xt = xt;
+                    if (ar2.base) { m->expanded.push_back(&L->w); m->expand_bytes += n_tiles * nq * 256 * sizeof(uint4); }
+                    if (fill && (launch_q4_expand_build(L->w, xt, m->ctx->stream) != hipSuccess || hipStreamSynchronize(m->ctx->stream) != hipSuccess))
+                        return setfail("q4_expand_build failed");
+                }
             }
             return true;
         }
@@ -1106,13 +1126,13 @@
         for (int i = 0; i < ne; i++) {
             EncLayer& L = m->enc[i]; std::string p = std::string(ENC_PFX ".transformer.layers.") + std::to_string(i);
             L.attn_norm = f32(p + ".attention_norm.weight"); L.ffn_norm = f32(p + ".ffn_norm.weight");
-            if (!lin({p + ".attention.wq.weight", p + ".attention.wk.weight", p + ".attention.wv.weight"}, false, &L.wqkv, q4)) return false;
+            if (!lin({p + ".attention.wq.weight", p + ".attention.wk.weight", p + ".attention.wv.weight"}, false, &L.wqkv, q4, true, true)) return false;
             const int64_t hq = L.wqkv.w.N / 3;
             L.wqkv.bias = bias_cat({{p + ".attention.wq.bias", hq}, {"", hq}, {p + ".attention.wv.bias", hq}});
-            if (!lin({p + ".attention.wo.weight"}, false, &L.wo, q4)) return false;
+            if (!lin({p + ".attention.wo.weight"}, false, &L.wo, q4, true, true)) return false;
             L.wo.bias = bias_cat({{p + ".attention.wo.bias", L.wo.w.N}});
             if (!lin({p + ".feed_forward.w1.weight", p + ".feed_forward.w3.weight"}, true, &L.w13, q4)) return false;
-            if (!lin({p + ".feed_forward.w2.weight"}, false, &L.w2, q4)) return false;
+            if (!lin({p + ".feed_forward.w2.weight"}, false, &L.w2, q4, true, true)) return false;
             L.w2.bias = bias_cat({{p + ".feed_forward.w2.bias", L.w2.w.N}});
         }
         m->enc_norm = f32(ENC_PFX ".transformer.norm.weight");
@@ -1177,8 +1197,9 @@
 }
 extern "C" int32_t vox_model_free(vox_model* m) { model_release(m); return VOX_OK; }
 
-static int32_t model_build(vox_ctx* ctx, const TensorSource* src_in, bool q4, bool layout_only, vox_model** out) {
+static int32_t model_build(vox_ctx* ctx, const TensorSource* src_in, bool q4, bool layout_only, vox_model** out, int expand = -1 ) {
     vox_model* m = new vox_model(); m->ctx = ctx;
+    { const char* e = knob_str("VOX_ENC_EXPAND"); m->enc_expand = expand >= 0 ? expand != 0 : !(e && e[0] == '0'); }
     RecordingSource rec(src_in); const TensorSource* src = &rec;
     std::map<std::string, bool> fmt_cache;
     Loader plan{m, src, Arena{}, false}; plan.fmt_cache = &fmt_cache;
@@ -1256,10 +1277,17 @@
     for (int gi = 0; gi < 4; gi++) if (m->engb_state[gi]) out[3] += engb_state_bytes();
     return VOX_OK;
 }
+extern "C" int32_t vox_model_memory_ex(const vox_model* m, uint64_t* out, int32_t cap) {
+    ARGCHK(m && out && cap >= 4, "bad argument");
+    VOXCHK(vox_model_memory(m, out));
+    for (int i = 4; i < cap; i++) out[i] = i == 4 ? m->expand_bytes : 0;
+    return VOX_OK;
+}
 extern "C" int32_t vox_model_arena(const vox_model* m, void** p, uint64_t* n) { ARGCHK(m && p && n, "null argument"); *p = m->arena; *n = m->arena_primary_bytes; return VOX_OK; }
 extern "C" int32_t vox_model_arena_finalize(vox_model* m) {
     ARGCHK(m, "null argument"); VOXCHK(ctx_bind(m->ctx));
     for (Q4W* w : m->tiled) HIPCHK(launch_q4_tile_build(*w, const_cast<uint4*>(w->qt), const_cast<uint16_t*>(w->st), m->ctx->stream));
+    for (Q4W* w : m->expanded) HIPCHK(launch_q4_expand_build(*w, const_cast<uint4*>(w->xt), m->ctx->stream));
     HIPCHK(hipStreamSynchronize(m->ctx->stream));
     m->eng_ready = false; m->eng_offline.cache = nullptr;
     prefix_release(m);
@@ -1275,7 +1303,7 @@
     VOXCHK(ctx_bind(dst_ctx));
     ManifestSource ms; ms.m = &src->manifest;
     vox_model* d = nullptr;
-    VOXCHK(model_build(dst_ctx, &ms, true, true, &d));
+    VOXCHK(model_build(dst_ctx, &ms, true, true, &d, src->enc_expand ? 1 : 0));
     if (d->arena_primary_bytes != src->arena_primary_bytes || d->arena_bytes != src->arena_bytes) { model_release(d); return fail(VOX_ERR_INVALID, "internal: replica arena layout differs from the source's"); }
     hipError_t e = src->ctx->device == dst_ctx->device ? hipMemcpyAsync(d->arena, src->arena, src->arena_primary_bytes, hipMemcpyDeviceToDevice, dst_ctx->stream)
                                                        : hipMemcpyPeerAsync(d->arena, dst_ctx->device, src->arena, src->ctx->device, src->arena_primary_bytes, dst_ctx->stream);
diff --git a/voxtral-mini-realtime-rs_amd/csrc/vox_kernels.h b/voxtral-mini-realtime-rs_amd/csrc/vox_kernels.h
--- a/voxtral-mini-realtime-rs_amd/csrc/vox_kernels.h
+++ b/voxtral-mini-realtime-rs_amd/csrc/vox_kernels.h
@@ -17,6 +17,7 @@
     int N, K, nb;
     int fmt;
     const uint4* qt = nullptr; const uint16_t* st = nullptr;
+    const uint4* xt = nullptr;
 };
 enum WFmt { WFMT_Q4_0 = 0, WFMT_BF16 = 1, WFMT_BF16X2 = 2, WFMT_F32 = 3 };
 
@@ -73,6 +74,7 @@
 size_t q4_wide_planes_bytes(const Q4W& w, int mt, const WidePlan& pl);
 hipError_t launch_q4_wide(const GemmParams& p, int epi, hipStream_t s);
 hipError_t launch_q4_tile_build(Q4W w, uint4* qt, uint16_t* st, hipStream_t s);
+hipError_t launch_q4_expand_build(Q4W w, uint4* xt, hipStream_t s);
 hipError_t launch_q4_gemm(const GemmParams& p, int epi, hipStream_t s, bool* fused_rope = nullptr);
 hipError_t launch_dense2_gemm(const GemmParams& p, int epi, hipStream_t s);
 hipError_t launch_transpose(const float* in, int R, int C, float* out, hipStream_t s);
@@ -131,7 +133,9 @@
 void attn_form_counts(unsigned long long out[ATTN_FORM_COUNT]);
 enum GemmForm { GEMM_FORM_GEMV_R1, GEMM_FORM_GEMV_R2, GEMM_FORM_GEMV_R4, GEMM_FORM_DENSE_GEMV, GEMM_FORM_SKINNY, GEMM_FORM_SKINNY_MT, GEMM_FORM_SKINNY_MT2, GEMM_FORM_XF_ROWS,
                 GEMM_FORM_SPLITK_FINISH, GEMM_FORM_TILE_11, GEMM_FORM_TILE_12, GEMM_FORM_TILE_21, GEMM_FORM_TILE_22, GEMM_FORM_TILE_21_TB, GEMM_FORM_TILE_22_TB, GEMM_FORM_K32,
-                GEMM_FORM_BIG, GEMM_FORM_BIG_ROPE, GEMM_FORM_DENSE2, GEMM_FORM_WIDE, GEMM_FORM_COUNT };
+                GEMM_FORM_BIG, GEMM_FORM_BIG_ROPE, GEMM_FORM_DENSE2, GEMM_FORM_WIDE,
+                GEMM_FORM_TILE_21_X, GEMM_FORM_TILE_22_X,
+                GEMM_FORM_COUNT };
 void gemm_form_counts(unsigned long long out[GEMM_FORM_COUNT]);
 
 hipError_t launch_conv1d_gelu(const float* in, int Cin, int L, const float* w, const float* b, int Cout, float* out,
diff --git a/voxtral-mini-realtime-rs_amd/csrc/vox_kernels.hip b/voxtral-mini-realtime-rs_amd/csrc/vox_kernels.hip
--- a/voxtral-mini-realtime-rs_amd/csrc/vox_kernels.hip
+++ b/voxtral-mini-realtime-rs_amd/csrc/vox_kernels.hip
@@ -827,7 +827,8 @@
         ws[t] = FMT == WFMT_Q4_0 ? p.w.sc + row * nb : nullptr;
         wd16[t] = p.w.qs + row * nb * 4 + wg;
         const size_t T = (size_t)min((n0 >> 4) + wave * NT + t, ((N + 15) >> 4) - 1);
-        wqt[t] = TB ? p.w.qt + T * nq * 64 + lane : nullptr;
+        wqt[t] = TB == 1 ? p.w.qt + T * nq * 64 + lane : nullptr;
+        if (TB == 2) wd16[t] = p.w.xt + T * nq * 256 + lane;
     }
     f32x4 acc[NT][MT];
 #pragma unroll
@@ -844,7 +845,8 @@
     }                                                                                                          \
     _Pragma("unroll") for (int t = 0; t < NT; t++) {                                                           \
         if (FMT == WFMT_Q4_0) {                                                                                \
-            if (TB) { const uint4 w4 = ld_nt_u4(wqt[t] + (size_t)64 * (Q_)); wd[t][0] = w4.x; wd[t][1] = w4.y; wd[t][2] = w4.z; wd[t][3] = w4.w; } \
+            if (TB == 2) { _Pragma("unroll") for (int j = 0; j < 4; j++) wdv[t][j] = wd16[t][(size_t)256 * (Q_) + 64 * j]; } \
+            else if (TB) { const uint4 w4 = ld_nt_u4(wqt[t] + (size_t)64 * (Q_)); wd[t][0] = w4.x; wd[t][1] = w4.y; wd[t][2] = w4.z; wd[t][3] = w4.w; } \
             else { _Pragma("unroll") for (int j = 0; j < 4; j++) wd[t][j] = wq[t][(size_t)(4 * (Q_) + j) * 4]; } \
             wsc[t] = *reinterpret_cast<const uint2*>(ws[t] + 4 * (Q_));                                        \
         } else {                                                                                               \
@@ -882,7 +884,7 @@
         for (int j = 0; j < 4; j++) {
 #pragma unroll
             for (int t = 0; t < NT; t++) {
-                const bf16x8 bw = as_bf16x8(FMT == WFMT_Q4_0 ? q4_dword_to_bf16x8(cwd[t][j]) : cwdv[t][j]);
+                const bf16x8 bw = as_bf16x8(FMT == WFMT_Q4_0 && TB != 2 ? q4_dword_to_bf16x8(cwd[t][j]) : cwdv[t][j]);
                 float d = 1.0f;
                 if (FMT == WFMT_Q4_0) {
                     const uint32_t pr = (j & 2) ? csc[t].y : csc[t].x;
@@ -949,6 +951,22 @@
             for (int j = 0; j < 4; j++) st[(tq * 16 + (lane & 15)) * 4 + j] = n < w.N ? w.sc[(size_t)n * w.nb + 4 * q + j] : (uint16_t)0;
         }
     }
+}
+__global__ void q4_expand_build_kernel(Q4W w, uint4* __restrict__ xt, int n_tiles) {
+    const int nq = w.nb >> 2;
+    const long total = (long)n_tiles * nq * 256;
+    for (long i = (long)blockIdx.x * blockDim.x + threadIdx.x; i < total; i += (long)gridDim.x * blockDim.x) {
+        const int lane = (int)(i & 63), j = (int)((i >> 6) & 3); const long tq = i >> 8; const int q = (int)(tq % nq), T = (int)(tq / nq);
+        const int g = lane >> 4, n = T * 16 + (lane & 15);
+        const uint32_t d = n < w.N ? reinterpret_cast<const uint32_t*>(w.qs)[((size_t)n * w.nb + 4 * q + j) * 4 + g] : 0x88888888u;
+        xt[i] = q4_dword_to_bf16x8(d);
+    }
+}
+hipError_t launch_q4_expand_build(Q4W w, uint4* xt, hipStream_t s) {
+    if (w.fmt != WFMT_Q4_0 || w.nb % 4 || !w.qs || !xt) return hipErrorInvalidValue;
+    const int n_tiles = (w.N + 15) / 16;
+    q4_expand_build_kernel<<<dim3(2048), dim3(256), 0, s>>>(w, xt, n_tiles);
+    return hipGetLastError();
 }
 hipError_t launch_q4_tile_build(Q4W w, uint4* qt, uint16_t* st, hipStream_t s) {
     if (w.nb % 4) return hipErrorInvalidValue;
@@ -2192,7 +2210,7 @@
     const size_t lds = (size_t)2 * 2 * 4 * MT * 64 * sizeof(uint4);
 #define VOX_E(E_) case E_: { auto kern = q4_gemm_kernel<MT, NT, E_, FMT, TB>; static DevOnce done;      \
         hipError_t e = ensure_dyn_lds(kern, lds, &done); if (e != hipSuccess) return e;                       \
-        gemm_form_note(TB ? (NT == 2 ? GEMM_FORM_TILE_22_TB : GEMM_FORM_TILE_21_TB) : MT == 1 ? (NT == 2 ? GEMM_FORM_TILE_12 : GEMM_FORM_TILE_11) : (NT == 2 ? GEMM_FORM_TILE_22 : GEMM_FORM_TILE_21)); \
+        gemm_form_note(TB == 2 ? (NT == 2 ? GEMM_FORM_TILE_22_X : GEMM_FORM_TILE_21_X) : TB ? (NT == 2 ? GEMM_FORM_TILE_22_TB : GEMM_FORM_TILE_21_TB) : MT == 1 ? (NT == 2 ? GEMM_FORM_TILE_12 : GEMM_FORM_TILE_11) : (NT == 2 ? GEMM_FORM_TILE_22 : GEMM_FORM_TILE_21)); \
         kern<<<grid, dim3(256), lds, s>>>(p); break; }
     switch (epi) { VOX_E(EPI_STORE) VOX_E(EPI_RESID) VOX_E(EPI_GELU) VOX_E(EPI_SWIGLU) default: return hipErrorInvalidValue; }
 #undef VOX_E
@@ -2219,6 +2237,7 @@
     if (wgs(mt, 2) < 256) nt = 1;
     if (FMT == WFMT_Q4_0 && p.w.qt && p.w.st && mt == 2) {
         if (wgs(2, 2) >= 128) nt = 2;
+        if (p.w.xt) return nt == 2 ? gemm_launch_mn<2, 2, WFMT_Q4_0, 2>(p, epi, s) : gemm_launch_mn<2, 1, WFMT_Q4_0, 2>(p, epi, s);
         return nt == 2 ? gemm_launch_mn<2, 2, WFMT_Q4_0, 1>(p, epi, s) : gemm_launch_mn<2, 1, WFMT_Q4_0, 1>(p, epi, s);
     }
 #define VOX_MN(M_, N_) if (mt == M_ && nt == N_) return gemm_launch_mn<M_, N_, FMT>(p, epi, s)
diff --git a/voxtral-mini-realtime-rs_amd/gguf.py b/voxtral-mini-realtime-rs_amd/gguf.py
--- a/voxtral-mini-realtime-rs_amd/gguf.py
+++ b/voxtral-mini-realtime-rs_amd/gguf.py
@@ -184,6 +184,9 @@
         out = np.empty(self._shape, dtype=np.float32)
         check(lib().vox_q4_tensor_dequantize(self.ctx.h, self.h, _ptr(out)))
         return out
+
+    def debug_expand(self, on=True):
+        check(lib().vox_debug_q4_expand(self.h, 1 if on else 0))
 
     def close(self):
         if self.h:
@@ -477,7 +480,7 @@
         v = (C.c_int32 * 4)(); check(lib().vox_model_prefix_info(self.h, v)); return {"built": bool(v[0]), "encoder_rows": v[1], "decoder_positions": v[2], "bytes": v[3]}
 
     def memory(self):
-        v = (C.c_uint64 * 4)(); check(lib().vox_model_memory(self.h, v)); return {"arena": v[0], "arena_primary": v[1], "engine_stream": v[2], "engine_state": v[3]}
+        v = (C.c_uint64 * 5)(); check(lib().vox_model_memory_ex(self.h, v, 5)); return {"arena": v[0], "arena_primary": v[1], "engine_stream": v[2], "engine_state": v[3], "enc_expand": v[4]}
 
     def set_batch_engine(self, on=None):
         a = C.c_int32(); n = C.c_uint64()
```

Measured after the change: 1500, median of 5. About the same (+0.3%).
